# KTH-RPL/neural_graph_mapping

Hardware: AMD Instinct MI355X
Metric: ray-samples/sec (train step: fwd+loss+bwd+Adam, 4096 rays x 128 samples per GPU) (higher is better)
Workload: dtype f32 via 3xbf16 split, fp32 accumulate (hidden-layer matrix products, forward and backward); everything else f32; 1 GPU; M1: 8 fields x 512 rays x (64 coarse + 64 depth-guided) samples per GPU, Fourier(64,raw)+2x64 MLP, nrgbd compositing, NRGBD intrinsics; fields_per_gpu=8, rays_per_field=512, samples_per_ray=128, ranks_seen=1, spin_up_steps=200, jitter=in-kernel Philox, launch=hipGraph replay

## Files before the change

### include/ngm_hip.h

```cpp
#ifndef NGM_HIP_H
#define NGM_HIP_H

#include <stdint.h>

#ifdef __cplusplus
extern "C" {
#endif

#define NGM_ABI_VERSION 11
#define NGM_MAX_LAYERS 4
#define NGM_NUM_LOSS_SUMS 16

enum ngm_status {
  NGM_OK = 0,
  NGM_E_INVALID = -1,
  NGM_E_UNSUPPORTED = -2,
  NGM_E_WORKSPACE = -3,
  NGM_E_HIP = -4
};

enum ngm_encoding { NGM_ENC_NONE = 0, NGM_ENC_FOURIER = 1, NGM_ENC_NERF = 2, NGM_ENC_PERMUTO = 3, NGM_ENC_TRIPLANE = 4 };
enum ngm_triplane_mode { NGM_TRI_SUM = 0, NGM_TRI_PRODUCT = 1, NGM_TRI_CONCAT = 2 };
enum ngm_skip_mode { NGM_SKIP_NO = 0, NGM_SKIP_ADD = 1, NGM_SKIP_CONCAT = 2 };
enum ngm_matmul_mode { NGM_MATMUL_F32 = 0, NGM_MATMUL_BF16X3 = 1, NGM_MATMUL_AUTO = 2 };
// ... 429 lines not shown
                   int32_t width, int32_t height, float fx, float fy, float cx, float cy, float near, float far, float* depth,
                   void* stream);
int ngm_mesh_visibility(const float* verts, int64_t num_verts, const float* c2w, int64_t num_poses, int32_t width, int32_t height,
                        float fx, float fy, float cx, float cy, const float* depth, float eps, int64_t num_frustum_poses,
                        int32_t* in_frustum, int32_t* observed, void* stream);

int64_t ngm_mesh_subdivide_workspace(int64_t num_faces);
int ngm_mesh_subdivide_count(const float* verts, int64_t num_verts, const int64_t* faces, int64_t num_faces, double max_edge,
                             int32_t max_iter, void* workspace, int64_t workspace_bytes, int64_t* totals_dev, void* stream);
int ngm_mesh_subdivide_emit(const float* verts, int64_t num_verts, const int64_t* faces, int64_t num_faces, const float* attrs,
                            int32_t num_channels, const void* workspace, int64_t new_vertices, int64_t out_faces, float* out_verts,
                            int64_t* out_faces_idx, float* out_attrs, int64_t* out_parent, void* stream);

int64_t ngm_mesh_vertex_normals_workspace(int64_t num_verts);
int ngm_mesh_vertex_normals(const float* verts, int64_t num_verts, const int64_t* faces, int64_t num_faces, float* normals,
                            void* workspace, int64_t workspace_bytes, void* stream);
int64_t ngm_icp_point_to_plane_workspace(int64_t num_target, int64_t num_source);
int ngm_icp_point_to_plane(const float* source, int64_t num_source, const float* target, const float* target_normals,
                           int64_t num_target, double threshold, int32_t max_iteration, double relative_fitness,
                           double relative_rmse, const double* init, double* state, void* workspace, int64_t workspace_bytes,
                           void* stream);

int64_t ngm_image_metrics_workspace(int32_t batch, int32_t height, int32_t width, int32_t crop);
int ngm_image_metrics(const float* pred, const float* target, int32_t batch, int32_t height, int32_t width, int32_t crop,
                      double* out, void* workspace, int64_t workspace_bytes, void* stream);

#define NGM_COVER_MAX_NEW 65536
typedef struct ngm_cover_depth_args {
  const float* depth;
  const float* c2w;
  const float* shift;
  const float* field_positions;
  const int64_t* field_ids;
  float* new_positions;
  int32_t* counts;
  int32_t pixel_stride;
  int32_t rows, num_active;
  int32_t height, width;
  int32_t max_new;
  float fx, fy, cx, cy;
  float radius, cell;
} ngm_cover_depth_args;
int64_t ngm_cover_depth_workspace(int32_t height, int32_t width, int32_t num_active, int32_t max_new);
int ngm_cover_depth(const ngm_cover_depth_args* a, void* workspace, int64_t workspace_bytes, void* stream);
int ngm_cover_depth_counters(int32_t height, int32_t width, int32_t num_active, int32_t max_new, void* workspace, int32_t* out5,
                             void* stream);

enum ngm_kernel_id {
  NGM_K_RENDER_FWD = 0,
  NGM_K_STASH_BWD = 1,
  NGM_K_FIELD_BWD = 2,
  NGM_K_GRAD_REDUCE = 3,
  NGM_K_ADAM = 4,
  NGM_K_POINTS_FWD = 5,
  NGM_K_COMPOSITE_FWD = 6,
  NGM_K_COMPOSITE_BWD = 7,
  NGM_K_HASH_GRAD = 8,
  NGM_K_HASH_REDUCE = 9,
  NGM_K_LOSS_REDUCE = 10,
  NGM_K_KNN_ASSIGN = 11,
  NGM_K_KNN_EVAL = 12,
  NGM_K_SAMPLER = 13,
  NGM_K_COUNT = 14
};
int ngm_profile_enable(int32_t on);
int ngm_profile_reset(void);
int ngm_profile_read(int32_t kernel_id, double* total_ms, int64_t* launches);

int ngm_debug_phase_cycles(unsigned long long* out528);
int ngm_debug_fwd_phase_cycles(unsigned long long* out528);

int ngm_debug_last_bwd_variant(void);
int ngm_debug_last_matmul(int which);
int ngm_debug_last_fwd_one_tile(void);
int ngm_debug_last_comp_fused(void);
int ngm_debug_disable_fused_comp(int on);
int ngm_debug_stash_mode(int mode);
int ngm_debug_last_stash_mode(void);
int ngm_debug_plan_bwd(const ngm_field_cfg* fcfg, const ngm_render_cfg* rcfg, int32_t F, int64_t n, int32_t guided,
                       int32_t stash_offered, int32_t seeds_written, int32_t* out5);
int ngm_debug_plan_fwd(const ngm_field_cfg* fcfg, const ngm_render_cfg* rcfg, int32_t surface, int32_t F, int64_t n, int32_t guided,
                       int32_t* out12);

#define NGM_MAX_PEERS 8
typedef struct ngm_peer_exchange {
  int32_t world, rank;
  void* mailbox[NGM_MAX_PEERS];
  unsigned long long* seq;
  int32_t* status;
} ngm_peer_exchange;
int64_t ngm_peer_mailbox_bytes(void);
int ngm_peer_alloc(int64_t bytes, void** ptr);
int ngm_peer_free(void* ptr);
int ngm_ipc_export(void* ptr, unsigned char handle[64]);
int ngm_ipc_open(const unsigned char handle[64], void** ptr);
int ngm_ipc_close(void* ptr);
int ngm_loss_exchange(const ngm_peer_exchange* px, float* loss_sums , void* stream);
double ngm_peer_set_timeout(double seconds);

#ifdef __cplusplus
}
#endif
#endif
```

### neural_graph_mapping_amd/_capi.py

```python
import ctypes as C
import os

HERE = os.path.dirname(os.path.abspath(__file__))
LIB_PATH = os.environ.get("NGM_LIB_PATH") or os.path.join(HERE, "lib", "libngm_hip.so")

NGM_MAX_LAYERS = 4
NGM_NUM_LOSS_SUMS = 16
ENC = {"none": 0, "fourier": 1, "nerf": 2, "permuto": 3, "triplane": 4}
TRI = {"sum": 0, "product": 1, "concat": 2}
SCALE = {"no": 0, "unit_ball": 1, "unit_cube": 2}
GEO = {"nrgbd": 0, "occupancy": 1, "density": 2, "neus": 3}
PHOTO = {"l1": 0, "l2": 1, "gaussian_nll": 2}
DEPTH = {"huber": 0, "gaussian_nll": 1, "laplacian_nll": 2}
LS = dict(PHOTO_SUM=0, PHOTO_CNT=1, DEPTH_SUM=2, DEPTH_CNT=3, FS_SUM=4, FS_CNT=5, TSDF_SUM=6,
          TSDF_CNT=7, TERM_SUM=8, TERM_CNT=9, PHOTO_L1_SUM=10)

f32p = C.c_void_p
LArr = C.c_void_p * (NGM_MAX_LAYERS + 1)
SArr = C.c_int64 * (NGM_MAX_LAYERS + 1)


class FieldCfg(C.Structure):
    _fields_ = [("encoding", C.c_int32), ("dim_enc", C.c_int32), ("raw_coords", C.c_int32),
                ("num_octaves", C.c_int32), ("start_octave", C.c_int32), ("num_layers", C.c_int32),
# ... 265 lines not shown
    L.ngm_render_eval_knn_workspace.argtypes = [P(RenderCfg), i32, i32, i32]
    L.ngm_render_eval_knn_workspace.restype = i64
    L.ngm_target_visibility.argtypes = [P(Keyframes), i32, vp, i32, vp, f32, vp, vp, vp]
    L.ngm_target_rays.argtypes = [P(Keyframes), i32, i32, vp, f32, vp, vp, vp, P(TargetOut), vp]
    L.ngm_target_visibility.restype = C.c_int
    L.ngm_target_rays.restype = C.c_int
    L.ngm_target_sv_intersect.argtypes = [i32, i64, vp, vp, f32, vp, vp]
    L.ngm_target_sv_intersect.restype = C.c_int
    L.ngm_target_sv_rays.argtypes = [i32, i32, vp, f32, vp, vp, vp, i32, i32, f32, f32, f32, f32, P(TargetOut), vp]
    L.ngm_target_sv_rays.restype = C.c_int
    L.ngm_target_sample_mv_workspace.argtypes = [i32, i32, i32, i32]
    L.ngm_target_sample_mv_workspace.restype = i64
    L.ngm_target_sample_mv.argtypes = [P(Keyframes), P(TargetSample), P(TargetOut), vp, i64, vp]
    L.ngm_target_sample_mv.restype = C.c_int
    L.ngm_target_sample_mv_live_workspace.argtypes = [i32, i32, i32, i32]
    L.ngm_target_sample_mv_live_workspace.restype = i64
    L.ngm_target_sample_mv_live.argtypes = [P(Keyframes), P(TargetSample), P(TargetLive), P(TargetOut), vp, i64, vp]
    L.ngm_target_sample_mv_live.restype = C.c_int
    L.ngm_target_observed_fields_workspace.argtypes = [i32, i32]
    L.ngm_target_observed_fields_workspace.restype = i64
    L.ngm_target_observed_fields.argtypes = [P(ObservedFields), vp, i64, vp]
    L.ngm_target_observed_fields.restype = C.c_int
    L.ngm_field_counts_add.argtypes = [vp, vp, i32, vp, i32, vp]
    L.ngm_field_counts_add.restype = C.c_int
    L.ngm_fields_append.argtypes = [P(FieldsAppendArgs), vp]
    L.ngm_fields_append.restype = C.c_int
    L.ngm_fields_repose.argtypes = [P(FieldsReposeArgs), vp]
    L.ngm_fields_repose.restype = C.c_int
    L.ngm_target_sample_mv_grow_workspace.argtypes = [i32, i32, i32, i32]
    L.ngm_target_sample_mv_grow_workspace.restype = i64
    L.ngm_target_sample_mv_grow.argtypes = [P(Keyframes), P(TargetSample), P(TargetLive), vp, P(TargetOut), vp, i64, vp]
    L.ngm_target_sample_mv_grow.restype = C.c_int
    L.ngm_target_observed_fields_grow_workspace.argtypes = [i32, i32]
    L.ngm_target_observed_fields_grow_workspace.restype = i64
    L.ngm_target_observed_fields_grow.argtypes = [P(ObservedFields), vp, vp, i64, vp]
    L.ngm_target_observed_fields_grow.restype = C.c_int
    L.ngm_marching_cubes_workspace.argtypes = [i32, i32, i32]
    L.ngm_marching_cubes_workspace.restype = i64
    L.ngm_marching_cubes_count.argtypes = [vp, i32, i32, i32, f32, vp, vp, i64, vp]
    L.ngm_marching_cubes_emit.argtypes = [vp, i32, i32, i32, f32, vp, i64, vp, i64, vp, i64, vp]
    L.ngm_marching_cubes_tables.argtypes = [vp, vp]
    for name in ("ngm_marching_cubes_count", "ngm_marching_cubes_emit", "ngm_marching_cubes_tables"):
        getattr(L, name).restype = C.c_int
    L.ngm_surface_sample_workspace.argtypes = [i64]
    L.ngm_surface_sample_workspace.restype = i64
    L.ngm_surface_sample.argtypes = [vp, i64, vp, i64, i64, C.c_uint64, vp, vp, vp, i64, vp]
    L.ngm_surface_sample.restype = C.c_int
    L.ngm_nearest_point_workspace.argtypes = [i64, i64]
    L.ngm_nearest_point_workspace.restype = i64
    L.ngm_nearest_point.argtypes = [vp, i64, vp, i64, vp, vp, vp, i64, vp]
    L.ngm_nearest_point.restype = C.c_int
    L.ngm_mesh_depth.argtypes = [vp, i64, vp, i64, vp, i64, i32, i32, f32, f32, f32, f32, f32, f32, vp, vp]
    L.ngm_mesh_depth.restype = C.c_int
    L.ngm_mesh_visibility.argtypes = [vp, i64, vp, i64, i32, i32, f32, f32, f32, f32, vp, f32, i64, vp, vp, vp]
    L.ngm_mesh_visibility.restype = C.c_int
    L.ngm_mesh_subdivide_workspace.argtypes = [i64]
    L.ngm_mesh_subdivide_workspace.restype = i64
    L.ngm_mesh_subdivide_count.argtypes = [vp, i64, vp, i64, C.c_double, i32, vp, i64, vp, vp]
    L.ngm_mesh_subdivide_count.restype = C.c_int
    L.ngm_mesh_subdivide_emit.argtypes = [vp, i64, vp, i64, vp, i32, vp, i64, i64, vp, vp, vp, vp, vp]
    L.ngm_mesh_subdivide_emit.restype = C.c_int
    L.ngm_mesh_vertex_normals_workspace.argtypes = [i64]
    L.ngm_mesh_vertex_normals_workspace.restype = i64
    L.ngm_mesh_vertex_normals.argtypes = [vp, i64, vp, i64, vp, vp, i64, vp]
    L.ngm_mesh_vertex_normals.restype = C.c_int
    L.ngm_icp_point_to_plane_workspace.argtypes = [i64, i64]
    L.ngm_icp_point_to_plane_workspace.restype = i64
    L.ngm_icp_point_to_plane.argtypes = [vp, i64, vp, vp, i64, C.c_double, i32, C.c_double, C.c_double, vp, vp, vp, i64, vp]
    L.ngm_icp_point_to_plane.restype = C.c_int
    L.ngm_image_metrics_workspace.argtypes = [i32, i32, i32, i32]
    L.ngm_image_metrics_workspace.restype = i64
    L.ngm_image_metrics.argtypes = [vp, vp, i32, i32, i32, i32, vp, vp, i64, vp]
    L.ngm_image_metrics.restype = C.c_int
    L.ngm_cover_depth_workspace.argtypes = [i32, i32, i32, i32]
    L.ngm_cover_depth_workspace.restype = i64
    L.ngm_cover_depth.argtypes = [P(CoverDepthArgs), vp, i64, vp]
    L.ngm_cover_depth.restype = C.c_int
    L.ngm_cover_depth_counters.argtypes = [i32, i32, i32, i32, vp, P(i32), vp]
    L.ngm_cover_depth_counters.restype = C.c_int
    L.ngm_debug_plan_bwd.argtypes = [P(FieldCfg), P(RenderCfg), i32, i64, i32, i32, i32, P(i32)]
    L.ngm_debug_plan_bwd.restype = C.c_int
    L.ngm_debug_plan_fwd.argtypes = [P(FieldCfg), P(RenderCfg), i32, i32, i64, i32, P(i32)]
    L.ngm_debug_plan_fwd.restype = C.c_int
    L.ngm_profile_enable.argtypes = [i32]
    L.ngm_profile_read.argtypes = [i32, P(C.c_double), P(i64)]
    for name in ("ngm_profile_enable", "ngm_profile_reset", "ngm_profile_read"):
        getattr(L, name).restype = C.c_int
    for name in ("ngm_sample_rays", "ngm_field_eval_fwd", "ngm_field_eval_bwd", "ngm_composite_fwd",
                 "ngm_composite_bwd", "ngm_render_fwd", "ngm_render_bwd", "ngm_render_bwd_seeded",
                 "ngm_render_read_samples", "ngm_adam_sparse", "ngm_field_eval_knn", "ngm_device_info"):
        getattr(L, name).restype = C.c_int
    _lib = L
    return L


EXPORTED = ["ngm_abi_version", "ngm_last_error", "ngm_device_info", "ngm_permuto_fill_scales", "ngm_sample_rays", "ngm_sample_rays_world", "ngm_sample_rays_weighted",
            "ngm_composite_fwd_packed",
            "ngm_field_eval_fwd", "ngm_encode_fwd", "ngm_encode_bwd", "ngm_encode_bwd_workspace", "ngm_field_eval_bwd", "ngm_field_eval_bwd_workspace",
            "ngm_field_eval_stash_bytes", "ngm_field_eval_fwd_train", "ngm_field_eval_bwd_stash",
            "ngm_composite_fwd", "ngm_composite_bwd", "ngm_render_workspace", "ngm_render_fwd",
            "ngm_render_bwd", "ngm_render_bwd_adam", "ngm_render_bwd_seeded", "ngm_render_bwd_seeded_vars", "ngm_render_read_samples", "ngm_adam_sparse",
            "ngm_field_eval_knn", "ngm_field_eval_knn_workspace", "ngm_grid_eval_knn", "ngm_grid_eval_knn_workspace", "ngm_render_eval_knn", "ngm_render_eval_knn_workspace", "ngm_adam_sparse_multi", "ngm_step_advance", "ngm_profile_enable", "ngm_profile_reset", "ngm_profile_read",
            "ngm_debug_phase_cycles", "ngm_debug_fwd_phase_cycles", "ngm_debug_last_bwd_variant", "ngm_debug_last_matmul", "ngm_debug_last_fwd_one_tile", "ngm_debug_last_comp_fused", "ngm_debug_disable_fused_comp", "ngm_debug_stash_mode", "ngm_debug_last_stash_mode", "ngm_debug_plan_bwd", "ngm_debug_plan_fwd", "ngm_target_visibility", "ngm_target_rays", "ngm_target_sv_intersect", "ngm_target_sv_rays",
            "ngm_target_sample_mv_workspace", "ngm_target_sample_mv",
            "ngm_target_sample_mv_live_workspace", "ngm_target_sample_mv_live", "ngm_target_observed_fields_workspace",
            "ngm_target_observed_fields", "ngm_field_counts_add",
            "ngm_fields_append", "ngm_fields_repose", "ngm_target_sample_mv_grow_workspace", "ngm_target_sample_mv_grow",
            "ngm_target_observed_fields_grow_workspace", "ngm_target_observed_fields_grow",
            "ngm_render_fwd_counted", "ngm_render_bwd_counted", "ngm_render_bwd_adam_counted",
            "ngm_peer_mailbox_bytes", "ngm_peer_alloc", "ngm_peer_free", "ngm_ipc_export", "ngm_ipc_open", "ngm_ipc_close", "ngm_loss_exchange", "ngm_peer_set_timeout",
            "ngm_marching_cubes_workspace", "ngm_marching_cubes_count", "ngm_marching_cubes_emit", "ngm_marching_cubes_tables",
            "ngm_surface_sample_workspace", "ngm_surface_sample", "ngm_nearest_point_workspace", "ngm_nearest_point",
            "ngm_mesh_depth", "ngm_mesh_visibility",
            "ngm_mesh_subdivide_workspace", "ngm_mesh_subdivide_count", "ngm_mesh_subdivide_emit",
            "ngm_mesh_vertex_normals_workspace", "ngm_mesh_vertex_normals", "ngm_icp_point_to_plane_workspace", "ngm_icp_point_to_plane",
            "ngm_image_metrics_workspace", "ngm_image_metrics",
            "ngm_cover_depth_workspace", "ngm_cover_depth", "ngm_cover_depth_counters"]

NO_GRAD_PARAMS = frozenset({"_encoding.random_shift_per_level"})

KERNEL_IDS = dict(render_fwd=0, stash_bwd=1, field_bwd=2, grad_reduce=3, adam=4, points_fwd=5, composite_fwd=6,
                  composite_bwd=7, hash_grad=8, hash_reduce=9, loss_reduce=10, knn_assign=11, knn_eval=12, sampler=13)


NGM_OK, NGM_E_INVALID, NGM_E_UNSUPPORTED, NGM_E_WORKSPACE, NGM_E_HIP = 0, -1, -2, -3, -4


class NgmError(RuntimeError):

    def __init__(self, msg, code=None):
        super().__init__(msg)
        self.code = code


def check(rc, what=""):
    if rc != 0:
        msg = lib().ngm_last_error().decode(errors="replace")
        raise NgmError(f"{what} failed with status {rc}: {msg}", code=int(rc))


SKIP = {"no": 0, "add": 1, "concat": 2}
STASH = {"full": 0, "half": 1}
HASH_ATOMICS = {"exact": 0, "float": 1}
MATMUL = {"f32": 0, "bf16x3": 1, "auto": 2}


def field_cfg(encoding="fourier", dim_enc=64, raw_coords=True, num_octaves=8, start_octave=0,
              num_layers=2, dim_hidden=None, dim_out=4, scale_mode="unit_cube", field_radius=1.0,
              nr_levels=16, nr_feat_per_level=2, log2_hashmap_size=12, coarsest_scale=1.0, finest_scale=1e-4,
              skip_mode="no", matmul_mode="f32", resolution=32, num_components=64, tri_mode="sum"):
    if skip_mode not in SKIP:
        raise NotImplementedError(f"skip_mode={skip_mode!r}: 'no', 'add' and 'concat' have kernels; the reference's own "
                                  "constructor raises for 'rezero' (models.py:131-132)")
    if encoding == "nerf":
        dim_enc = 6 * num_octaves
    if encoding == "none":
        dim_enc = 3
    if encoding == "permuto":
        dim_enc = nr_levels * nr_feat_per_level
    if encoding == "triplane":
        dim_enc = num_components * (3 if tri_mode == "concat" else 1)
    if dim_hidden is None:
        dim_hidden = dim_enc
    fc = FieldCfg(ENC[encoding], dim_enc, int(bool(raw_coords)), num_octaves, start_octave,
                  num_layers, dim_hidden, dim_out, SCALE[scale_mode], float(field_radius), nr_levels,
                  nr_feat_per_level, log2_hashmap_size, float(coarsest_scale), float(finest_scale))
    fc.skip_mode = SKIP[skip_mode]
    fc.matmul_mode = MATMUL[matmul_mode]
    fc.tri_resolution, fc.tri_mode = int(resolution), TRI[tri_mode]
    if encoding == "permuto":
        import math
        import numpy as np
        sig = np.geomspace(coarsest_scale, finest_scale, num=nr_levels)
        for lvl in range(min(nr_levels, 16)):
            for i in range(3):
                fc.level_scale[3 * lvl + i] = np.float32((1.0 / math.sqrt((i + 1) * (i + 2))) / sig[lvl])
    return fc


def param_names(fc: FieldCfg):
    names = []
    if fc.encoding == ENC["fourier"]:
        names.append("_encoding._linear.weight")
    if fc.encoding == ENC["permuto"]:
        names += ["_encoding.lattice_values", "_encoding.random_shift_per_level"]
    if fc.encoding == ENC["triplane"]:
# ... 77 lines not shown
```

### neural_graph_mapping_amd/csrc/ngm_api.hip

```cpp
#include <hip/hip_runtime.h>
#include <stdio.h>
#include <stdlib.h>
#include <string.h>

#include "../../include/ngm_hip.h"
#include "ngm_launch.h"
#include "ngm_workspace.h"

int ngm_launch_sampler_weighted(const ngm_render_cfg* rc, const ngm_rays* rays, int S, int B, const float* boundaries,
                                const float* weights, float* points_cam, float* distances, float* dirs, hipStream_t st);
int ngm_launch_sampler(const ngm_render_cfg* rc, const ngm_rays* rays, int S, float* points_cam, float* distances,
                       float* dirs, float* points_world, hipStream_t st);
int ngm_launch_loss_values(const ngm_render_cfg* rc, const float* sums, float* out, hipStream_t st);
int ngm_launch_loss_reduce(const float* partials, int nblocks, float* sums, uint64_t* counter, hipStream_t st);
int ngm_launch_neus_sd_grad(const float* d_isd_rays, int F, int R, const float* neus_sd, int64_t sd_stride,
                            const int64_t* field_index, float* d_sd, hipStream_t st);
int ngm_launch_read_stash(const float4* sa, const float2* sb, int64_t n, float* geoms, float* dists, hipStream_t st);
int ngm_launch_adam(float* param, float* m, float* v, int64_t stride, const float* grad, int64_t gstride, int F, int64_t numel,
                    const AdamHyper& h, hipStream_t st);
int ngm_launch_adam_multi(const ngm_adam_tensor* tensors, int n, int F, const AdamHyper& h, int64_t* advance_step,
                          uint64_t* advance_offset, hipStream_t st, const int32_t* num_active = nullptr);
int ngm_launch_step_advance(int64_t* step_dev, uint64_t* off_dev, hipStream_t st);
int64_t ngm_mc_workspace_bytes(int nx, int ny, int nz);
int ngm_launch_mc_count(const float* vol, int nx, int ny, int nz, float iso, int64_t* counts, void* workspace,
// ... 658 lines not shown

int ngm_encode_fwd(const ngm_field_cfg* fcfg, const ngm_params* params, int32_t F, int64_t P, const float* points,
                   const float* field_pos, const float* field_quat, float* out, void* stream) {
  int rc = check_field_cfg(fcfg, false);
  if (rc) return rc;
  rc = check_params(fcfg, params);
  if (rc) return rc;
  if (!points || !out || F < 1 || P < 0) return fail(NGM_E_INVALID, "ngm_encode_fwd: bad argument");
  if ((field_pos == nullptr) != (field_quat == nullptr)) return fail(NGM_E_INVALID, "pos/quat must both be given");
  if (P == 0) return NGM_OK;
  rc = ngm_launch_encode_points(*fcfg, *params, F, P, points, field_pos, field_quat, out, (hipStream_t)stream);
  if (rc) return fail(rc, "ngm_encode_fwd: encoding not available as a standalone stage (triplane)");
  return check_launch("ngm_encode_fwd");
}

static int64_t tri_numel(const ngm_field_cfg* fc) {
  const int64_t C = fc->tri_mode == NGM_TRI_CONCAT ? fc->dim_enc / 3 : fc->dim_enc;
  return 3 * C * fc->tri_resolution * fc->tri_resolution;
}
static void hash_scratch_layout(const ngm_field_cfg* fc, int F, int64_t P, FieldBwdArgs& a, WsArena& ws) {
  if (fc->encoding == NGM_ENC_TRIPLANE) { a.tri_numel = tri_numel(fc); a.tri_acc = ws.take<long long>((int64_t)F * a.tri_numel); return; }
  if (fc->encoding != NGM_ENC_PERMUTO) return;
  a.hash_dE = ws.take<float2>((int64_t)fc->nr_levels * F * P);
  a.hash_xyz = ws.take<float4>((int64_t)F * P);
  a.hash_part = ws.take<float>((int64_t)F * fc->nr_levels * 8 * 2 * ((int64_t)1 << fc->log2_hashmap_size));
}

static void encode_bwd_layout(const ngm_field_cfg* fc, int F, int64_t P, float** fourier_part, FieldBwdArgs& a, WsArena& ws) {
  if (fc->encoding == NGM_ENC_FOURIER) *fourier_part = ws.take<float>(ngm_encode_bwd_fourier_scratch(F, P) / 4);
  if (fc->encoding == NGM_ENC_PERMUTO) hash_scratch_layout(fc, F, P, a, ws);
}
int64_t ngm_encode_bwd_workspace(const ngm_field_cfg* fcfg, int32_t F, int64_t P) {
  if (!fcfg || F < 1 || P < 0) return NGM_E_INVALID;
  float* fourier_part;
  return ws_bytes(encode_bwd_layout, fcfg, F, P, &fourier_part, FieldBwdArgs());
}

int ngm_encode_bwd(const ngm_field_cfg* fcfg, const ngm_params* params, int32_t F, int64_t P, const float* points,
                   const float* field_pos, const float* field_quat, const float* d_enc, const ngm_grads* grads, void* workspace,
                   int64_t workspace_bytes, void* stream) {
  int rc = check_field_cfg(fcfg, false);
  if (rc) return rc;
  rc = check_params(fcfg, params);
  if (rc) return rc;
  if (!points || !d_enc || !grads || F < 1 || P < 0) return fail(NGM_E_INVALID, "ngm_encode_bwd: bad argument");
  if ((field_pos == nullptr) != (field_quat == nullptr)) return fail(NGM_E_INVALID, "pos/quat must both be given");
  if (fcfg->encoding == NGM_ENC_TRIPLANE)
    return fail(NGM_E_UNSUPPORTED, "ngm_encode_bwd: the triplane encoding has no standalone backward stage (ngm_field_eval_bwd)");
  if (fcfg->encoding != NGM_ENC_PERMUTO && fcfg->encoding != NGM_ENC_FOURIER) return NGM_OK;
  FieldBwdArgs a;
  memset(&a, 0, sizeof(a));
  float* fourier_part = nullptr;
  WsArena ws(workspace);
  encode_bwd_layout(fcfg, F, P, &fourier_part, a, ws);
  if (!workspace || !ws.covers(workspace_bytes)) return fail(NGM_E_WORKSPACE, "ngm_encode_bwd: workspace too small");
  hipStream_t st = (hipStream_t)stream;
  if (fcfg->encoding == NGM_ENC_FOURIER) {
    if (!grads->enc_w) return fail(NGM_E_INVALID, "ngm_encode_bwd: grads->enc_w is NULL");
    if (P == 0) {
      const int64_t n = (int64_t)(fcfg->dim_enc - (fcfg->raw_coords ? 3 : 0)) * 3;
      for (int f = 0; f < F; ++f) (void)hipMemsetAsync(grads->enc_w + f * grads->enc_w_stride, 0, 4 * (size_t)n, st);
      return check_launch("ngm_encode_bwd");
    }
    rc = ngm_launch_encode_bwd_fourier(*fcfg, *params, F, P, points, field_pos, field_quat, d_enc, grads->enc_w, grads->enc_w_stride,
                                       fourier_part, st);
    if (rc) return fail(rc, "ngm_encode_bwd: launch failed");
    return check_launch("ngm_encode_bwd");
  }
  if (!grads->lattice) return fail(NGM_E_INVALID, "ngm_encode_bwd: grads->lattice is NULL");
  if (!ngm_hash_grad_takes(*fcfg)) return fail(NGM_E_UNSUPPORTED, "ngm_encode_bwd: table size not supported by the table-gradient kernel");
  a.fc = *fcfg; a.pr = *params; a.F = F; a.P = P;
  a.lattice_grad = grads->lattice; a.lattice_grad_stride = grads->lattice_stride;
  if (P == 0) {
    const int64_t n = (int64_t)fcfg->nr_levels * ((int64_t)1 << fcfg->log2_hashmap_size) * 2;
    for (int f = 0; f < F; ++f) (void)hipMemsetAsync(grads->lattice + f * grads->lattice_stride, 0, 4 * (size_t)n, st);
    return check_launch("ngm_encode_bwd");
  }
  rc = ngm_launch_encode_bwd_prep_hash(*fcfg, *params, F, P, points, field_pos, field_quat, d_enc, a.hash_dE, a.hash_xyz, st);
  if (!rc) rc = ngm_launch_hash_grad(a, st);
  if (rc) return fail(rc, "ngm_encode_bwd: table size not supported by the table-gradient kernel");
  return check_launch("ngm_encode_bwd");
}

static int64_t param_pad(const ngm_field_cfg* fc) {
  int64_t e, w[NGM_MAX_LAYERS + 1], b[NGM_MAX_LAYERS + 1];
  return align_up(ngm_param_offsets(fc, &e, w, b), 64);
}

static void field_eval_bwd_layout(const ngm_field_cfg* fc, int64_t P, FieldBwdArgs& a, WsArena& ws) {
  a.partials = ws.take<float>((int64_t)a.F * a.blocks_per_field * a.p_pad + 64);
  hash_scratch_layout(fc, a.F, P, a, ws);
}
int64_t ngm_field_eval_bwd_workspace(const ngm_field_cfg* fcfg, int32_t F, int64_t P) {
  if (check_field_cfg(fcfg)) return NGM_E_INVALID;
  FieldBwdArgs a = FieldBwdArgs();
  int64_t per;
  a.F = F; a.p_pad = param_pad(fcfg);
  plan_bwd(F, P, &per, &a.blocks_per_field);
  return ws_bytes(field_eval_bwd_layout, fcfg, P, a);
}

static BwdPlan plan_points(const ngm_field_cfg* fc, int32_t F, int64_t P, bool stash_offered) { return plan_mlp_bwd(fc, BwdAsk{nullptr, F, P, false, stash_offered}); }
static float* field_eval_stash_layout(const ngm_field_cfg* fc, int32_t F, int64_t P, int64_t* layer_stride, WsArena& ws) {
  *layer_stride = align_up((int64_t)F * P, 32) * 64 + 2048;
  return ws.take<float>(fc->num_layers * *layer_stride + 16);
}
int64_t ngm_field_eval_stash_bytes(const ngm_field_cfg* fcfg, int32_t F, int64_t P) {
  if (check_field_cfg(fcfg) || F < 1 || P < 0) return NGM_E_INVALID;
  if (P == 0 || !plan_points(fcfg, F, P, true).stash_kind) return 0;
  int64_t stride;
  return ws_bytes(field_eval_stash_layout, fcfg, F, P, &stride);
}
static int field_eval_fwd(const ngm_field_cfg* fcfg, const ngm_params* params, int32_t F, int64_t P,
                          const float* points, const float* field_pos, const float* field_quat, float* out, bool stash_offered,
                          void* stash, int64_t stash_bytes, void* stream) {
  int rc = check_field_cfg(fcfg);
  if (rc) return rc;
  rc = check_params(fcfg, params);
  if (rc) return rc;
  if (!points || !out || F < 1 || P < 0) return fail(NGM_E_INVALID, "ngm_field_eval_fwd: bad argument");
  if ((field_pos == nullptr) != (field_quat == nullptr)) return fail(NGM_E_INVALID, "pos/quat must both be given");
  if (P == 0) return NGM_OK;
  FwdAsk ask;
  ask.surface = NGM_FWD_POINTS; ask.F = F; ask.n = P;
  const FwdPlan plan = plan_fwd(fcfg, ask);
  if (plan.status) return fail(plan.status, plan.why);
  PointsFwdArgs a;
  memset(&a, 0, sizeof(a));
  a.fc = *fcfg; a.pr = *params; a.F = F; a.P = P; a.points = points; a.pos = field_pos; a.quat = field_quat; a.out = out;
  if (stash_offered) {
    if (ngm_field_eval_stash_bytes(fcfg, F, P) <= 0) return fail(NGM_E_UNSUPPORTED, "ngm_field_eval_fwd_train: no stash-reading backward for this configuration (ngm_field_eval_stash_bytes == 0): use ngm_field_eval_fwd / ngm_field_eval_bwd");
    WsArena ss(stash);
    a.act = field_eval_stash_layout(fcfg, F, P, &a.act_layer_stride, ss);
    if (!stash || !ss.covers(stash_bytes)) return fail(NGM_E_WORKSPACE, "ngm_field_eval_fwd_train: stash too small (ngm_field_eval_stash_bytes)");
  }
  a.per_block = plan.per_block;
  rc = ngm_launch_points_fwd(a, plan, (hipStream_t)stream);
  if (rc) return fail(rc, no_instance);
  g_last_fwd[NGM_FWD_POINTS] = plan;
  return check_launch("ngm_field_eval_fwd");
}
int ngm_field_eval_fwd(const ngm_field_cfg* fcfg, const ngm_params* params, int32_t F, int64_t P, const float* points,
                       const float* field_pos, const float* field_quat, float* out, void* stream) {
  return field_eval_fwd(fcfg, params, F, P, points, field_pos, field_quat, out, false, nullptr, 0, stream);
}
int ngm_field_eval_fwd_train(const ngm_field_cfg* fcfg, const ngm_params* params, int32_t F, int64_t P, const float* points,
                             const float* field_pos, const float* field_quat, float* out, void* stash, int64_t stash_bytes,
                             void* stream) {
  return field_eval_fwd(fcfg, params, F, P, points, field_pos, field_quat, out, true, stash, stash_bytes, stream);
}

static int field_eval_bwd(const ngm_field_cfg* fcfg, const ngm_params* params, int32_t F, int64_t P,
                          const float* points, const float* field_pos, const float* field_quat, const float* d_out,
                          const ngm_grads* grads, bool stash_offered, const void* stash, int64_t stash_bytes, void* workspace,
                          int64_t workspace_bytes, void* stream) {
  int rc = check_field_cfg(fcfg);
  if (rc) return rc;
  rc = check_params(fcfg, params);
  if (rc) return rc;
  if (!points || !d_out || !grads || F < 1 || P < 1) return fail(NGM_E_INVALID, "ngm_field_eval_bwd: bad argument");
  if ((field_pos == nullptr) != (field_quat == nullptr)) return fail(NGM_E_INVALID, "pos/quat must both be given");
  const BwdPlan plan = plan_points(fcfg, F, P, stash_offered);
  if (plan.status) return fail(plan.status, plan.why);
  FieldBwdArgs a;
  memset(&a, 0, sizeof(a));
  if (stash_offered) {
    if (!plan.stash_kind) return fail(NGM_E_UNSUPPORTED, "ngm_field_eval_bwd_stash: no stash-reading backward for this configuration");
    WsArena ss(stash);
    a.act = field_eval_stash_layout(fcfg, F, P, &a.act_layer_stride, ss);
    if (!stash || !ss.covers(stash_bytes)) return fail(NGM_E_WORKSPACE, "ngm_field_eval_bwd_stash: stash too small");
  }
  a.F = F; a.blocks_per_field = plan.blocks_per_field; a.p_pad = param_pad(fcfg);
  WsArena ws(workspace);
  field_eval_bwd_layout(fcfg, P, a, ws);
  if (!ws.covers(workspace_bytes) || !workspace) return fail(NGM_E_WORKSPACE, "workspace too small");
  hipStream_t st = (hipStream_t)stream;
  a.fc = *fcfg; a.pr = *params; a.F = F; a.P = P; a.points = points; a.pos = field_pos; a.quat = field_quat;
  a.d_out = reinterpret_cast<const float4*>(d_out);
  a.per_block = plan.per_block;
  rc = check_enc_grads(fcfg, grads, a);
  if (rc) return rc;
  if (a.tri_acc) (void)hipMemsetAsync(a.tri_acc, 0, (size_t)F * a.tri_numel * 8, st);
  rc = launch_mlp_bwd(plan, a, st);
  if (rc) return rc;
  if (fcfg->encoding == NGM_ENC_TRIPLANE) { ngm_launch_tri_finish(a, st); rc = check_launch("ngm_tri_finish"); if (rc) return rc; }
  if (fcfg->encoding == NGM_ENC_PERMUTO) {
    rc = ngm_launch_hash_grad(a, st);
    if (rc) return fail(rc, "permutohedral backward: hash table too large for the LDS-staged scatter");
    rc = check_launch("ngm_hash_grad");
    if (rc) return rc;
  }
  GradReduceArgs g;
  memset(&g.adam, 0, sizeof(g.adam));
  g.fc = *fcfg; g.gr = *grads; g.F = F; g.blocks_per_field = a.blocks_per_field; g.partials = a.partials; g.p_pad = a.p_pad;
  ngm_launch_grad_reduce(g, st);
  return check_launch("ngm_grad_reduce");
}
int ngm_field_eval_bwd(const ngm_field_cfg* fcfg, const ngm_params* params, int32_t F, int64_t P, const float* points,
                       const float* field_pos, const float* field_quat, const float* d_out, const ngm_grads* grads,
                       void* workspace, int64_t workspace_bytes, void* stream) {
  return field_eval_bwd(fcfg, params, F, P, points, field_pos, field_quat, d_out, grads, false, nullptr, 0, workspace, workspace_bytes, stream);
}
int ngm_field_eval_bwd_stash(const ngm_field_cfg* fcfg, const ngm_params* params, int32_t F, int64_t P, const float* points,
                             const float* field_pos, const float* field_quat, const float* d_out, const ngm_grads* grads,
                             const void* stash, int64_t stash_bytes, void* workspace, int64_t workspace_bytes, void* stream) {
  return field_eval_bwd(fcfg, params, F, P, points, field_pos, field_quat, d_out, grads, true, stash, stash_bytes, workspace, workspace_bytes, stream);
}

int ngm_composite_fwd(const ngm_render_cfg* cfg, int64_t N, int32_t S, const float* colors, const float* geoms,
                      const float* dists, const float* depths, const float* neus_isds, float* C, float* D, float* Cvar,
                      float* Dvar, float* term, float* weights, void* stream) {
  if (!cfg || !colors || !geoms || !dists || !depths || N < 0) return fail(NGM_E_INVALID, "ngm_composite_fwd: bad argument");
  if (N == 0) return NGM_OK;
  CompositeArgs a;
  memset(&a, 0, sizeof(a));
  a.rc = *cfg; a.N = N; a.S = S; a.colors = colors; a.geoms = geoms; a.dists = dists; a.depths = depths; a.isds = neus_isds;
  a.C = C; a.D = D; a.Cv = Cvar; a.Dv = Dvar; a.term = term; a.weights = weights;
  const int rc = ngm_launch_composite_fwd(a, (hipStream_t)stream);
  if (rc) return fail(rc, "ngm_composite_fwd: unsupported S (max 1024)");
  return check_launch("ngm_composite_fwd");
}

int ngm_composite_fwd_packed(const ngm_render_cfg* cfg, int64_t N, int32_t S, const float* field_out4, const float* dists,
                             const float* points_cam, float* rgbd, float* Cvar, float* Dvar, float* term, void* stream) {
  if (!cfg || !field_out4 || !dists || !points_cam || N < 0) return fail(NGM_E_INVALID, "ngm_composite_fwd_packed: bad argument");
  if (N == 0) return NGM_OK;
  CompositeArgs a;
  memset(&a, 0, sizeof(a));
  a.rc = *cfg; a.N = N; a.S = S; a.out4 = reinterpret_cast<const float4*>(field_out4); a.pcam = points_cam; a.dists = dists;
  a.rgbd = rgbd; a.Cv = Cvar; a.Dv = Dvar; a.term = term;
  const int rc = ngm_launch_composite_fwd(a, (hipStream_t)stream);
  if (rc) return fail(rc, "ngm_composite_fwd_packed: unsupported S (max 1024)");
  return check_launch("ngm_composite_fwd_packed");
}

int ngm_composite_bwd(const ngm_render_cfg* cfg, int64_t N, int32_t S, const float* colors, const float* geoms,
                      const float* dists, const float* depths, const float* neus_isds, const float* dC, const float* dD,
                      const float* dterm, float* d_colors, float* d_geoms, float* d_neus_isds, void* stream) {
  if (!cfg || !colors || !geoms || !dists || !depths || N < 0) return fail(NGM_E_INVALID, "ngm_composite_bwd: bad argument");
  if (N == 0) return NGM_OK;
  CompositeArgs a;
  memset(&a, 0, sizeof(a));
  a.rc = *cfg; a.N = N; a.S = S; a.colors = colors; a.geoms = geoms; a.dists = dists; a.depths = depths; a.isds = neus_isds;
  a.dC = dC; a.dD = dD; a.dterm = dterm; a.d_colors = d_colors; a.d_geoms = d_geoms; a.d_isds = d_neus_isds;
  const int rc = ngm_launch_composite_bwd(a, (hipStream_t)stream);
  if (rc) return fail(rc, "ngm_composite_bwd: S > 1024");
  return check_launch("ngm_composite_bwd");
}

struct RenderPlan {
  int S;
  FwdPlan fwd;
  BwdPlan bwd;
  int64_t p_pad;
  int64_t off_rayseed;
// ... 121 lines not shown
    a.raytab = reinterpret_cast<float*>(ws + p.off_raytab);
    if (has_tg) a.rayseed = reinterpret_cast<float*>(ws + p.off_rayseed);
    a.stashA = reinterpret_cast<float4*>(ws + p.off_stashA);
    a.stashB = reinterpret_cast<float2*>(ws + p.off_stashB);
    a.loss_partials = reinterpret_cast<float*>(ws + p.off_losspart);
    if (p.act_layer_stride) { a.act = reinterpret_cast<float*>(ws + p.off_act); a.act_layer_stride = p.act_layer_stride; }
    a.act_layers = p.bwd.half;
    static const bool timing = getenv("NGM_PHASE_TIMING") != nullptr;
    if (timing) {
      if (!g_debug_cycles_fwd) { (void)hipMalloc(&g_debug_cycles_fwd, NGM_FWD_DEBUG_WORDS * 8); (void)hipMemset(g_debug_cycles_fwd, 0, NGM_FWD_DEBUG_WORDS * 8); }
      a.debug_cycles = g_debug_cycles_fwd;
    }
  }
  e = ngm_launch_render_fwd(a, p.fwd, (hipStream_t)stream);
  if (e) return fail(e, no_instance);
  g_last_fwd[NGM_FWD_RENDER] = p.fwd;
  if (save) {
    note_forward_stash(workspace, p.bwd.half);
    note_forward_seeds(workspace, a.rayseed ? targets->rgbds : nullptr);
  }
  e = check_launch("ngm_render_fwd");
  if (e) return e;
  if (has_tg && loss_sums) {
    ngm_launch_loss_reduce(a.loss_partials, p.fwd.blocks, loss_sums,
                           (rays->philox_offset_autoinc && rays->philox_offset_dev) ? const_cast<uint64_t*>(rays->philox_offset_dev) : nullptr,
                           (hipStream_t)stream);
    e = check_launch("ngm_loss_reduce");
  }
  return e;
}
int ngm_render_fwd(const ngm_field_cfg* fcfg, const ngm_render_cfg* rcfg, const ngm_params* params, const ngm_rays* rays,
                   const ngm_targets* targets, const ngm_prediction* pred, float* loss_sums, void* workspace,
                   int64_t workspace_bytes, void* stream) {
  return render_fwd_impl(fcfg, rcfg, params, rays, targets, pred, loss_sums, workspace, workspace_bytes, stream, nullptr);
}
int ngm_render_fwd_counted(const ngm_field_cfg* fcfg, const ngm_render_cfg* rcfg, const ngm_params* params, const ngm_rays* rays,
                           const ngm_targets* targets, const ngm_prediction* pred, float* loss_sums, void* workspace,
                           int64_t workspace_bytes, void* stream, const int32_t* num_active) {
  const int e = check_counted("ngm_render_fwd_counted", fcfg, rcfg, num_active);
  if (e) return e;
  return render_fwd_impl(fcfg, rcfg, params, rays, targets, pred, loss_sums, workspace, workspace_bytes, stream, num_active);
}

static int render_bwd_common(const ngm_field_cfg* fcfg, const ngm_render_cfg* rcfg, const ngm_params* params,
                             const ngm_rays* rays, StashBwdArgs& sb, const ngm_grads* grads, void* workspace,
                             int64_t workspace_bytes, hipStream_t st, const GradAdam* adam = nullptr,
                             const GradAdam* lattice_adam = nullptr, bool* lattice_adam_applied = nullptr,
                             const int32_t* num_active = nullptr) {
  BwdAsk ask;
  ask.seeded = sb.seed_mode != 0; ask.rec_layers = forward_stash_layers(workspace); ask.seeds_written = forward_wrote_seeds_for(workspace, sb.tg.rgbds);
  FieldBwdArgs a;
  memset(&a, 0, sizeof(a));
  const RenderPlan p = plan_render(fcfg, rcfg, rays->F, rays->R, rays->gt != nullptr, true, ask, false, workspace, &a);
  if (p.bwd.status) return fail(p.bwd.status, p.bwd.why);
  if (!workspace || workspace_bytes < p.total) return fail(NGM_E_WORKSPACE, "render_bwd: workspace too small");
  const bool nll_loss = rcfg->photometric_mode == NGM_PHOTO_GAUSSIAN_NLL || rcfg->depth_mode != NGM_DEPTH_HUBER;
  if (nll_loss && sb.seed_mode == 0 && (!sb.pred.color_vars || !sb.pred.depth_vars))
    return fail(NGM_E_INVALID, "render_bwd: the *_nll loss modes need pred.color_vars and pred.depth_vars");
  char* ws = p.base;
  a.fc = *fcfg; a.pr = *params; a.F = rays->F; a.P = (int64_t)rays->R * p.S; a.S = p.S;
  a.num_active = num_active;
  int e = check_enc_grads(fcfg, grads, a);
  if (e) return e;
  sb.rc = *rcfg; sb.F = rays->F; sb.R = rays->R; sb.S = p.S;
  sb.num_active = num_active;
  if (!rays->gt) sb.rc.w_freespace = sb.rc.w_tsdf = 0.f;
  sb.stashA = reinterpret_cast<float4*>(ws + p.off_stashA);
  sb.stashB = reinterpret_cast<const float2*>(ws + p.off_stashB);
  sb.raytab = reinterpret_cast<const float*>(ws + p.off_raytab);
  const bool neus = rcfg->geometry_mode == NGM_GEO_NEUS;
  if (neus) {
    sb.neus_sd = params->neus_sd; sb.neus_sd_stride = params->neus_sd_stride; sb.field_index = params->field_index;
    sb.d_out = reinterpret_cast<float4*>(ws + p.off_dout);
    sb.d_isd_rays = reinterpret_cast<float*>(ws + p.off_disd);
  }
  if (sb.seed_mode == 0 && !sb.loss_sums) {
    sb.loss_partials = reinterpret_cast<const float*>(ws + p.off_losspart);
    sb.n_partials = p.fwd.blocks;
    sb.counter = (rays->philox_offset_autoinc && rays->philox_offset_dev)
                     ? reinterpret_cast<unsigned long long*>(const_cast<uint64_t*>(rays->philox_offset_dev)) : nullptr;
  }
  a.per_block = p.bwd.per_block; a.blocks_per_field = p.bwd.blocks_per_field;
  a.raytab = sb.raytab; a.stashB = sb.stashB; a.d_out = neus ? sb.d_out : sb.stashA;
  a.partials = reinterpret_cast<float*>(ws + p.off_gradpart); a.p_pad = p.p_pad;
  if (p.bwd.stash_kind) { a.act = reinterpret_cast<const float*>(ws + p.off_act); a.act_layer_stride = p.act_layer_stride; a.act_half = p.bwd.half; }
  if (p.bwd.fused_comp) {
    a.fused_comp = 1; a.rc = sb.rc;
    a.rayseed = reinterpret_cast<const float*>(ws + p.off_rayseed);
    a.loss_sums = sb.loss_sums; a.loss_partials = sb.loss_partials; a.n_partials = sb.n_partials;
    a.sums_out = sb.sums_out; a.loss_out = sb.loss_out; a.counter = sb.counter;
  } else {
    sb.xyz_out = a.hash_xyz;
    a.hash_xyz_ready = a.hash_xyz != nullptr;
    e = ngm_launch_stash_bwd(sb, st);
    if (e) return fail(e, "render_bwd: unsupported geometry mode");
    e = check_launch("ngm_stash_bwd");
    if (e) return e;
  }
  if (neus && grads->neus_sd)
    ngm_launch_neus_sd_grad(sb.d_isd_rays, rays->F, rays->R, params->neus_sd, params->neus_sd_stride, params->field_index,
                            grads->neus_sd, st);
  if (a.tri_acc) (void)hipMemsetAsync(a.tri_acc, 0, (size_t)a.F * a.tri_numel * 8, st);
  e = launch_mlp_bwd(p.bwd, a, st);
  if (e) return e;
  if (fcfg->encoding == NGM_ENC_TRIPLANE) { ngm_launch_tri_finish(a, st); e = check_launch("ngm_tri_finish"); if (e) return e; }
  GradReduceArgs g;
  memset(&g.adam, 0, sizeof(g.adam));
  if (adam) g.adam = *adam;
  g.num_active = num_active;
  g.fc = *fcfg; g.gr = *grads; g.F = rays->F; g.blocks_per_field = a.blocks_per_field; g.partials = a.partials; g.p_pad = a.p_pad;
  bool mlp_reduced = false;
  if (fcfg->encoding == NGM_ENC_PERMUTO) {
    if (lattice_adam) a.lattice_adam = *lattice_adam;
    e = ngm_launch_hash_grad(a, st, lattice_adam_applied, &g, &mlp_reduced);
    if (e == NGM_E_INVALID) return fail(e, "render_bwd_adam: adam tensors do not match the parameter segments");
    if (e) return fail(e, "permutohedral backward: hash table too large for the LDS-staged scatter");
    e = check_launch("ngm_hash_grad");
    if (e) return e;
  }
  if (mlp_reduced) return NGM_OK;
  if (ngm_launch_grad_reduce(g, st)) return fail(NGM_E_INVALID, "render_bwd_adam: adam tensors do not match the parameter segments");
  return check_launch("ngm_grad_reduce");
}

static int render_bwd_impl(const ngm_field_cfg* fcfg, const ngm_render_cfg* rcfg, const ngm_params* params, const ngm_rays* rays,
                           const ngm_targets* targets, const ngm_prediction* pred, const float* loss_sums, const ngm_grads* grads,
                           float* loss_out, void* workspace, int64_t workspace_bytes, void* stream, const int32_t* num_active) {
  int e = check_render(fcfg, rcfg, params, rays);
  if (e) return e;
  if (!targets || !targets->rgbds || !targets->depth_mask || !pred || !pred->rgbds || !pred->term_probs || !grads)
    return fail(NGM_E_INVALID, "render_bwd: NULL argument");
  StashBwdArgs sb;
  memset(&sb, 0, sizeof(sb));
  sb.seed_mode = 0; sb.tg = *targets; sb.pred = *pred; sb.loss_sums = loss_sums;
  sb.loss_out = loss_out;
  return render_bwd_common(fcfg, rcfg, params, rays, sb, grads, workspace, workspace_bytes, (hipStream_t)stream, nullptr, nullptr,
                           nullptr, num_active);
}
int ngm_render_bwd(const ngm_field_cfg* fcfg, const ngm_render_cfg* rcfg, const ngm_params* params, const ngm_rays* rays,
                   const ngm_targets* targets, const ngm_prediction* pred, const float* loss_sums, const ngm_grads* grads,
                   float* loss_out, void* workspace, int64_t workspace_bytes, void* stream) {
  return render_bwd_impl(fcfg, rcfg, params, rays, targets, pred, loss_sums, grads, loss_out, workspace, workspace_bytes, stream,
                         nullptr);
}
int ngm_render_bwd_counted(const ngm_field_cfg* fcfg, const ngm_render_cfg* rcfg, const ngm_params* params, const ngm_rays* rays,
                           const ngm_targets* targets, const ngm_prediction* pred, const float* loss_sums, const ngm_grads* grads,
                           float* loss_out, void* workspace, int64_t workspace_bytes, void* stream, const int32_t* num_active) {
  const int e = check_counted("ngm_render_bwd_counted", fcfg, rcfg, num_active);
  if (e) return e;
  return render_bwd_impl(fcfg, rcfg, params, rays, targets, pred, loss_sums, grads, loss_out, workspace, workspace_bytes, stream,
                         num_active);
}

static int render_bwd_adam_impl(const ngm_field_cfg* fcfg, const ngm_render_cfg* rcfg, const ngm_params* params, const ngm_rays* rays,
                                const ngm_targets* targets, const ngm_prediction* pred, const float* loss_sums, const ngm_grads* grads,
                                const ngm_adam_tensor* mlp_tensors, int32_t num_mlp_tensors, const ngm_adam_tensor* lattice_tensor,
                                const int64_t* field_index, int64_t step, int64_t* step_dev, float lr, float beta1, float beta2,
                                float eps, float weight_decay, float* loss_out, void* workspace, int64_t workspace_bytes,
                                void* stream, const int32_t* num_active) {
  int e = check_render(fcfg, rcfg, params, rays);
  if (e) return e;
  if (!targets || !targets->rgbds || !targets->depth_mask || !pred || !pred->rgbds || !pred->term_probs || !grads ||
      !mlp_tensors || num_mlp_tensors < 1 || (step < 1 && !step_dev))
    return fail(NGM_E_INVALID, "render_bwd_adam: bad argument");
  if ((fcfg->encoding == NGM_ENC_PERMUTO) != (lattice_tensor != nullptr))
    return fail(NGM_E_INVALID, "render_bwd_adam: lattice_tensor goes with the permutohedral encoding");
  StashBwdArgs sb;
// ... 434 lines not shown
      hipStreamSynchronize((hipStream_t)stream) != hipSuccess)
    return check_launch("ngm_cover_depth_counters") == NGM_OK ? fail(NGM_E_HIP, "ngm_cover_depth_counters: copy failed") : NGM_E_HIP;
  return NGM_OK;
}

static int hip_fail(hipError_t e, const char* what) {
  snprintf(g_err, sizeof(g_err), "%s: %s", what, hipGetErrorString(e));
  (void)hipGetLastError();
  return NGM_E_HIP;
}
int64_t ngm_peer_mailbox_bytes(void) { return 2 * NGM_MAX_PEERS * 16 * 8; }
int ngm_peer_alloc(int64_t bytes, void** ptr) {
  if (!ptr || bytes <= 0) return fail(NGM_E_INVALID, "ngm_peer_alloc: bad argument");
  const int e = ngm_peer_alloc_impl(bytes, ptr);
  return e ? hip_fail((hipError_t)e, "ngm_peer_alloc") : NGM_OK;
}
int ngm_peer_free(void* ptr) {
  const hipError_t e = hipFree(ptr);
  return e == hipSuccess ? NGM_OK : hip_fail(e, "ngm_peer_free");
}
int ngm_ipc_export(void* ptr, unsigned char handle[64]) {
  static_assert(sizeof(hipIpcMemHandle_t) == 64, "hipIpcMemHandle_t is 64 bytes");
  if (!ptr || !handle) return fail(NGM_E_INVALID, "ngm_ipc_export: NULL");
  hipIpcMemHandle_t h;
  const hipError_t e = hipIpcGetMemHandle(&h, ptr);
  if (e != hipSuccess) return hip_fail(e, "hipIpcGetMemHandle");
  memcpy(handle, &h, 64);
  return NGM_OK;
}
int ngm_ipc_open(const unsigned char handle[64], void** ptr) {
  if (!ptr || !handle) return fail(NGM_E_INVALID, "ngm_ipc_open: NULL");
  hipIpcMemHandle_t h;
  memcpy(&h, handle, 64);
  const hipError_t e = hipIpcOpenMemHandle(ptr, h, hipIpcMemLazyEnablePeerAccess);
  return e == hipSuccess ? NGM_OK : hip_fail(e, "hipIpcOpenMemHandle");
}
int ngm_ipc_close(void* ptr) {
  const hipError_t e = hipIpcCloseMemHandle(ptr);
  return e == hipSuccess ? NGM_OK : hip_fail(e, "hipIpcCloseMemHandle");
}
int ngm_debug_last_stash_mode(void) { return g_last_bwd.stash_kind ? g_last_bwd.half : -1; }
int ngm_debug_stash_mode(int mode) {
  const int prev = g_stash_override;
  if (mode >= 0 && mode <= 1) g_stash_override = mode;
  else if (mode == -2) g_stash_override = -1;
  return prev;
}

int ngm_debug_plan_bwd(const ngm_field_cfg* fcfg, const ngm_render_cfg* rcfg, int32_t F, int64_t n, int32_t guided,
                       int32_t stash_offered, int32_t seeds_written, int32_t* out5) {
  const int e = check_field_cfg(fcfg);
  if (e) return e;
  if (!out5 || F < 1 || n < 1 || (rcfg && n > INT32_MAX)) return fail(NGM_E_INVALID, "ngm_debug_plan_bwd: bad argument");
  BwdPlan bp;
  int fwd_matmul = -1;
  if (rcfg) {
    BwdAsk ask;
    ask.seeds_written = seeds_written != 0;
    const RenderPlan p = plan_render(fcfg, rcfg, F, (int)n, guided != 0, true, ask);
    bp = p.bwd;
    fwd_matmul = p.fwd.matmul;
  } else {
    bp = plan_points(fcfg, F, n, stash_offered != 0);
  }
  out5[0] = bp.variant; out5[1] = bp.fused_comp; out5[2] = bp.stash_kind; out5[3] = bp.stash_layers; out5[4] = fwd_matmul;
  return bp.status ? fail(bp.status, bp.why) : NGM_OK;
}

int ngm_debug_plan_fwd(const ngm_field_cfg* fcfg, const ngm_render_cfg* rcfg, int32_t surface, int32_t F, int64_t n, int32_t guided,
                       int32_t* out12) {
  const int e = check_field_cfg(fcfg);
  if (e) return e;
  if (!out12 || surface < NGM_FWD_RENDER || surface > NGM_FWD_KNN || (surface == NGM_FWD_RENDER) != (rcfg != nullptr) || F < 1 || n < 1 ||
      (rcfg && n > INT32_MAX))
    return fail(NGM_E_INVALID, "ngm_debug_plan_fwd: bad argument");
  FwdAsk ask;
  ask.surface = surface; ask.F = F; ask.n = n;
  const FwdPlan p = rcfg ? plan_render(fcfg, rcfg, F, (int)n, guided != 0, false).fwd : plan_fwd(fcfg, ask);
  const int32_t out[12] = {p.MI, p.MH, p.L, p.matmul, p.one_tile, p.waves, (int32_t)p.lds_bytes, p.neus, p.threads, p.rays_per_block, p.maxs, p.blocks};
  memcpy(out12, out, sizeof(out));
  return p.status ? fail(p.status, p.why) : NGM_OK;
}

double ngm_peer_set_timeout(double seconds) { return ngm_peer_set_timeout_impl(seconds); }

int ngm_loss_exchange(const ngm_peer_exchange* px, float* loss_sums, void* stream) {
  if (!px || !loss_sums || !px->seq || !px->status) return fail(NGM_E_INVALID, "ngm_loss_exchange: NULL");
  if (px->world < 1 || px->world > NGM_MAX_PEERS || px->rank < 0 || px->rank >= px->world)
    return fail(NGM_E_INVALID, "ngm_loss_exchange: 1 <= world <= 8, 0 <= rank < world");
  for (int p = 0; p < px->world; ++p)
    if (!px->mailbox[p]) return fail(NGM_E_INVALID, "ngm_loss_exchange: mailbox of a rank not mapped");
  ngm_launch_loss_exchange(*px, loss_sums, (hipStream_t)stream);
  return check_launch("ngm_loss_exchange");
}

}
```

### neural_graph_mapping_amd/csrc/ngm_bwd16.h

```cpp
#pragma once
#include "ngm_field.h"
#include "ngm_launch.h"

typedef float f32x4 __attribute__((ext_vector_type(4)));

#define WAVE_SYNC()                                        \
  do {                                                     \
    __builtin_amdgcn_fence(__ATOMIC_RELEASE, "wavefront"); \
    __builtin_amdgcn_wave_barrier();                       \
    __builtin_amdgcn_fence(__ATOMIC_ACQUIRE, "wavefront"); \
  } while (0)

#ifdef NGM_PHASE_TIMING
#define TICK_DECL                                                        \
  unsigned long long tacc[12] = {0, 0, 0, 0, 0, 0, 0, 0, 0, 0, 0, 0};    \
  unsigned long long tlast = __builtin_readcyclecounter();               \
  const unsigned long long tstart = tlast
#define TICK(k)                                                          \
  do {                                                                   \
    if (a.debug_cycles) {                                                \
      const unsigned long long now_ = __builtin_readcyclecounter();      \
      tacc[k] += now_ - tlast; tlast = __builtin_readcyclecounter();     \
    }                                                                    \
  } while (0)
// ... 405 lines not shown
    for (int r = 0; r < 4; ++r)
#pragma unroll
      for (int mi = 0; mi < TIN; ++mi) dX[mi] = mfma16(abuf[mo & 1][mi][r], dY[mo][r], dX[mi]);
    __builtin_amdgcn_sched_barrier(0);
  }
}

template <int TOUT, int TIN>
__device__ __forceinline__ void wgrad16(const float* __restrict__ dbuf, int dstr, const float* __restrict__ xbuf, int xstr,
                                        int lane, f32x4 (&acc)[TOUT][TIN]) {
  const int i = lane & 15, q = lane >> 4;
  const float* dl = dbuf + q * dstr + i;
  const float* xl = xbuf + q * xstr + i;
  float av[2][TOUT], bv[2][TIN];
#pragma unroll
  for (int mo = 0; mo < TOUT; ++mo) av[0][mo] = dl[16 * mo];
#pragma unroll
  for (int mi = 0; mi < TIN; ++mi) bv[0][mi] = xl[16 * mi];
#pragma unroll
  for (int t = 0; t < 4; ++t) {
    if (t + 1 < 4) {
#pragma unroll
      for (int mo = 0; mo < TOUT; ++mo) av[(t + 1) & 1][mo] = dl[4 * (t + 1) * dstr + 16 * mo];
#pragma unroll
      for (int mi = 0; mi < TIN; ++mi) bv[(t + 1) & 1][mi] = xl[4 * (t + 1) * xstr + 16 * mi];
    }
    __builtin_amdgcn_sched_barrier(0);
#pragma unroll
    for (int mo = 0; mo < TOUT; ++mo)
#pragma unroll
      for (int mi = 0; mi < TIN; ++mi) acc[mo][mi] = mfma16(av[t & 1][mo], bv[t & 1][mi], acc[mo][mi]);
    __builtin_amdgcn_sched_barrier(0);
  }
}

template <int T>
__device__ __forceinline__ float colsum16(const float* buf, int stride, int lane) {
  constexpr int NF = 16 * T, PARTS = (64 % NF == 0) ? 64 / NF : 1, PER = 16 / PARTS;
  if (lane >= NF * PARTS) return 0.f;
  const int fl = lane % NF, sp = lane / NF;
  float v[PER];
#pragma unroll
  for (int k = 0; k < PER; ++k) v[k] = buf[(sp * PER + k) * stride + fl];
#pragma unroll
  for (int w = PER / 2; w >= 1; w >>= 1)
#pragma unroll
    for (int k = 0; k < w; ++k) v[k] += v[k + w];
  return v[0];
}
template <int T, int NC>
__device__ __forceinline__ void outer16(const float* colbuf, int stride, const float* row4, int lane, float (&acc)[NC]) {
  constexpr int NF = 16 * T, PARTS = (64 % NF == 0) ? 64 / NF : 1, PER = 16 / PARTS;
  if (lane >= NF * PARTS) return;
  const int fl = lane % NF, sp = lane / NF;
  constexpr int BATCH = (PER < 8) ? PER : 8;
#pragma unroll
  for (int k0 = 0; k0 < PER; k0 += BATCH) {
    float h[BATCH]; float4 d[BATCH];
#pragma unroll
    for (int k = 0; k < BATCH; ++k) { const int s = sp * PER + k0 + k; h[k] = colbuf[s * stride + fl]; d[k] = *reinterpret_cast<const float4*>(row4 + 4 * s); }
#pragma unroll
    for (int k = 0; k < BATCH; ++k) {
      acc[0] = fmaf(d[k].x, h[k], acc[0]); acc[1] = fmaf(d[k].y, h[k], acc[1]); acc[2] = fmaf(d[k].z, h[k], acc[2]);
      if (NC > 3) acc[3] = fmaf(d[k].w, h[k], acc[3]);
    }
  }
}
template <int T>
__device__ __forceinline__ float fold_parts(float v) {
  constexpr int NF = 16 * T;
  if (NF <= 32) v += __shfl_down(v, 32, 64);
  if (NF <= 16) v += __shfl_down(v, 16, 64);
  return v;
}

template <int TI, int TH, int L, bool ENC_GRAD, int EPI_CH = 4>
__device__ __forceinline__ void bwd16_epilogue(const FieldBwdArgs& a, float* stage, f32x4 (&acc0)[TH][TI],
                                               f32x4 (&accH)[(L > 1) ? (L - 1) : 1][TH][TH], float (&dbh)[L],
                                               float (&dwo)[4], float (&dwf)[3], float (&dbo)[4]) {
  const int lane = threadIdx.x & 63, wave = threadIdx.x >> 6;
  int64_t enc_off, w_off[NGM_MAX_LAYERS + 1], b_off[NGM_MAX_LAYERS + 1];
  const int64_t ptot = ngm_param_offsets(&a.fc, &enc_off, w_off, b_off);
  (void)ptot;
  float* dst = a.partials + (int64_t)blockIdx.x * a.p_pad;
  const int D = a.fc.dim_enc, H = a.fc.dim_hidden;
  constexpr int NT0 = TH * TI, NTH = TH * TH, NT = NT0 + (L - 1) * NTH;
  constexpr int EPI_W = EPI_CH * 4 * 64;
#pragma unroll
  for (int t0 = 0; t0 < NT; t0 += EPI_CH) {
#pragma unroll
    for (int tt = 0; tt < EPI_CH; ++tt) {
      const int t = t0 + tt;
      if (t < NT) {
#pragma unroll
        for (int r = 0; r < 4; ++r) {
          float v;
          if (t < NT0) v = acc0[t / TI][t % TI][r];
          else v = accH[(t - NT0) / NTH][((t - NT0) % NTH) / TH][(t - NT0) % TH][r];
          stage[wave * EPI_W + (tt * 4 + r) * 64 + lane] = v;
        }
      }
    }
    __syncthreads();
    for (int e = threadIdx.x; e < EPI_W; e += B16_THREADS) {
      float s0 = 0.f;
#pragma unroll
      for (int w = 0; w < B16_WAVES; ++w) s0 += stage[w * EPI_W + e];
      const int t = t0 + (e >> 8), r = (e >> 6) & 3, jj = e & 15, qq = (e >> 4) & 3;
      if (t < NT) {
        int l, mo, mi, din;
        if (t < NT0) { l = 0; mo = t / TI; mi = t % TI; din = D; }
        else { const int u = t - NT0; l = 1 + u / NTH; mo = (u % NTH) / TH; mi = u % TH; din = H; }
        const int o = 16 * mo + 4 * qq + r, c = 16 * mi + jj;
        if (o < H && c < din) dst[w_off[l] + (int64_t)o * din + c] = s0;
      }
    }
    __syncthreads();
  }
#pragma unroll
  for (int l = 0; l < L; ++l) dbh[l] = fold_parts<TH>(dbh[l]);
#pragma unroll
  for (int c = 0; c < 4; ++c) dwo[c] = fold_parts<TH>(dwo[c]);
#pragma unroll
  for (int c = 0; c < 3; ++c) dwf[c] = fold_parts<TI>(dwf[c]);
#pragma unroll
  for (int c = 0; c < 4; ++c) dbo[c] = wave_sum(dbo[c]);
  constexpr int NV = L + 4 + 3 + 4;
  static_assert(NV * 64 <= EPI_W, "per-feature vectors must fit one staging round");
  {
    float* sw = stage + wave * EPI_W;
#pragma unroll
    for (int l = 0; l < L; ++l) sw[l * 64 + lane] = dbh[l];
#pragma unroll
    for (int c = 0; c < 4; ++c) sw[(L + c) * 64 + lane] = dwo[c];
#pragma unroll
    for (int c = 0; c < 3; ++c) sw[(L + 4 + c) * 64 + lane] = dwf[c];
#pragma unroll
    for (int c = 0; c < 4; ++c) sw[(L + 7 + c) * 64 + lane] = dbo[c];
  }
  __syncthreads();
  const bool fourier = ENC_GRAD && a.fc.encoding == NGM_ENC_FOURIER;
  const int n_raw = a.fc.raw_coords ? 3 : 0;
  for (int e = threadIdx.x; e < NV * 64; e += B16_THREADS) {
    float s0 = 0.f;
#pragma unroll
    for (int w = 0; w < B16_WAVES; ++w) s0 += stage[w * EPI_W + e];
    const int k = e >> 6, ln = e & 63;
    if (k < L) { if (ln < H) dst[b_off[k] + ln] = s0; }
    else if (k < L + 4) { if (ln < H) dst[w_off[L] + (int64_t)(k - L) * H + ln] = s0; }
    else if (k < L + 7) { if (fourier && ln < D && ln >= n_raw) dst[enc_off + (int64_t)(ln - n_raw) * 3 + (k - L - 4)] = s0; }
    else if (ln == 0) dst[b_off[L] + (k - L - 7)] = s0;
  }
  if (!fourier)
    for (int64_t p = enc_off + threadIdx.x; p < w_off[0]; p += B16_THREADS) dst[p] = 0.f;
}
```

### neural_graph_mapping_amd/csrc/ngm_field_bwd.hip

```cpp
#include <stdlib.h>
#include <string.h>
#include <algorithm>
#include "ngm_field.h"
#include "ngm_launch.h"

#define WAVE_SYNC()                                        \
  do {                                                     \
    __builtin_amdgcn_fence(__ATOMIC_RELEASE, "wavefront"); \
    __builtin_amdgcn_wave_barrier();                       \
    __builtin_amdgcn_fence(__ATOMIC_ACQUIRE, "wavefront"); \
  } while (0)

template <int MI, int MH, int L, bool CAT = false>
struct BwdLds {
  using LY = FieldLds<MI, MH, L, CAT>;
  static constexpr int STR_E = 32 * MI + 4;
  static constexpr int STR_H = 32 * MH + 4;
  static constexpr int STR_D = (STR_E > STR_H) ? STR_E : STR_H;
  static constexpr int X0 = 0;
  static constexpr int x_off(int l) { return l == 0 ? 0 : 32 * STR_E + (l - 1) * 32 * STR_H; }
  static constexpr int DBUF = 32 * STR_E + (L - 1) * 32 * STR_H;
  static constexpr int PBUF = DBUF + 32 * STR_D;
  static constexpr int OBUF = PBUF + 128;
  static constexpr int WAVE_TOTAL = OBUF + 128;
// ... 383 lines not shown
#pragma unroll
            for (int r = 0; r < 16; ++r) dY[mi][r] = (Xl[mi][r] > 0.f) ? dX[mi][r] : 0.f;
        }
      }
    }
  }

  __syncthreads();
  float* red = sm + LY::TOTAL;
  int64_t enc_off, w_off[NGM_MAX_LAYERS + 1], b_off[NGM_MAX_LAYERS + 1];
  const int64_t ptot = ngm_param_offsets(&a.fc, &enc_off, w_off, b_off);
  for (int64_t p = threadIdx.x; p < ptot; p += NGM_BLOCK) red[p] = 0.f;
  __syncthreads();
  const int D = a.fc.dim_enc, H = a.fc.dim_hidden;
  if (MH == 1) {
#pragma unroll
    for (int l = 0; l < L; ++l) dbh[l] += __shfl_down(dbh[l], 32, 64);
#pragma unroll
    for (int c = 0; c < 4; ++c) dwo[c] += __shfl_down(dwo[c], 32, 64);
  }
  if (MI == 1) {
#pragma unroll
    for (int c = 0; c < 3; ++c) dwf[c] += __shfl_down(dwf[c], 32, 64);
    if constexpr (CAT) {
#pragma unroll
      for (int c = 0; c < 4; ++c) dwoE[c] += __shfl_down(dwoE[c], 32, 64);
    }
  }
  const int DC = CAT ? H + D : H;
#pragma unroll
  for (int c = 0; c < 4; ++c) dbo[c] = wave_sum(dbo[c]);
  for (int w = 0; w < NGM_WAVES_PER_BLOCK; ++w) {
    if (wave == w) {
#pragma unroll
      for (int mo = 0; mo < MH; ++mo) {
#pragma unroll
        for (int r = 0; r < 16; ++r) {
          const int o = 32 * mo + frow(r, hi);
          if (o < H) {
#pragma unroll
            for (int mi = 0; mi < MI; ++mi) {
              const int i = 32 * mi + j;
              if (i < D) red[w_off[0] + (int64_t)o * D + i] += acc0[mo][mi][r];
            }
#pragma unroll
            for (int l = 1; l < L; ++l) {
#pragma unroll
              for (int mi = 0; mi < MH; ++mi) {
                const int i = 32 * mi + j;
                if (i < H) red[w_off[l] + (int64_t)o * DC + i] += accH[l - 1][mo][mi][r];
              }
              if constexpr (CAT) {
#pragma unroll
                for (int mi = 0; mi < MI; ++mi) {
                  const int i = 32 * mi + j;
                  if (i < D) red[w_off[l] + (int64_t)o * DC + H + i] += accE[l - 1][mo][mi][r];
                }
              }
            }
          }
        }
      }
      if (lane < 32 * MH && lane < H) {
#pragma unroll
        for (int l = 0; l < L; ++l) red[b_off[l] + lane] += dbh[l];
#pragma unroll
        for (int c = 0; c < 4; ++c) red[w_off[L] + (int64_t)c * DC + lane] += dwo[c];
      }
      if (CAT && lane < 32 * MI && lane < D) {
#pragma unroll
        for (int c = 0; c < 4; ++c) red[w_off[L] + (int64_t)c * DC + H + lane] += dwoE[c];
      }
      if (lane < 4) red[b_off[L] + lane] += (lane == 0 ? dbo[0] : lane == 1 ? dbo[1] : lane == 2 ? dbo[2] : dbo[3]);
      if (ENC_GRAD && a.fc.encoding == NGM_ENC_FOURIER) {
        const int n_raw = a.fc.raw_coords ? 3 : 0;
        if (lane < 32 * MI && lane < D && lane >= n_raw) {
#pragma unroll
          for (int c = 0; c < 3; ++c) red[enc_off + (int64_t)(lane - n_raw) * 3 + c] += dwf[c];
        }
      }
    }
    __syncthreads();
  }
  float* dst = a.partials + (int64_t)blockIdx.x * a.p_pad;
  for (int64_t p = threadIdx.x; p < ptot; p += NGM_BLOCK) dst[p] = red[p];
}

struct GradSeg { int64_t off, size; float* dst; int64_t stride; float* param; float* m; float* v; int64_t pstride; void* lp; int lp_dt; };
struct GradReduceK {
  int F, blocks_per_field, nseg;
  const float* partials;
  int64_t p_pad, ptot;
  GradSeg seg[2 * (NGM_MAX_LAYERS + 1) + 1];
  AdamHyper hyper;
  const int32_t* num_active;
};

template <bool COUNTED>
__global__ void __launch_bounds__(256) k_grad_reduce(GradReduceK a) {
  __shared__ float part[4][64];
  const int f = blockIdx.y, q = threadIdx.x >> 6, l = threadIdx.x & 63;
  if constexpr (COUNTED) {
    if (f >= *a.num_active) return;
  }
  const int64_t p = (int64_t)blockIdx.x * 64 + l;
  int seg = -1;
  int64_t so = 0;
  float pv = 0.f, m0 = 0.f, v0 = 0.f;
  AdamCoef co = {0.f, 1.f};
  const bool adam = q == 0 && p < a.ptot;
  if (adam) {
    for (int k = 0; k < a.nseg; ++k)
      if (p >= a.seg[k].off && p < a.seg[k].off + a.seg[k].size) { seg = k; break; }
    if (seg >= 0 && a.seg[seg].param) {
      const int64_t row = a.hyper.field_index ? a.hyper.field_index[f] : f;
      so = row * a.seg[seg].pstride + (p - a.seg[seg].off);
      pv = a.seg[seg].param[so]; m0 = a.seg[seg].m[so]; v0 = a.seg[seg].v[so];
    }
  }
  const float* src = a.partials + (int64_t)f * a.p_pad + p;
  const int64_t cs = (int64_t)a.F * a.p_pad;
  int c = q;
  float v8[8] = {0.f, 0.f, 0.f, 0.f, 0.f, 0.f, 0.f, 0.f};
  const bool pre = p < a.ptot && c + 28 < a.blocks_per_field;
  if (pre) {
#pragma unroll
    for (int j = 0; j < 8; ++j) v8[j] = src[(c + 4 * j) * cs];
  }
  if (adam && seg >= 0 && a.seg[seg].param) {
    const double step = (double)(a.hyper.step_dev ? *a.hyper.step_dev : a.hyper.step);
    co = adam_coef(a.hyper.lr, a.hyper.beta1, a.hyper.beta2, step);
  }
  float s = 0.f;
  if (pre) {
#pragma unroll
    for (int j = 0; j < 8; ++j) s += v8[j];
    c += 32;
  }
  if (p < a.ptot) {
#pragma unroll 1
    for (; c + 28 < a.blocks_per_field; c += 32) {
      float v[8];
#pragma unroll
      for (int j = 0; j < 8; ++j) v[j] = src[(c + 4 * j) * cs];
#pragma unroll
      for (int j = 0; j < 8; ++j) s += v[j];
    }
#pragma unroll 1
    for (; c + 12 < a.blocks_per_field; c += 16) {
      const float v0_ = src[c * cs], v1 = src[(c + 4) * cs], v2 = src[(c + 8) * cs], v3 = src[(c + 12) * cs];
      s += v0_; s += v1; s += v2; s += v3;
    }
    for (; c < a.blocks_per_field; c += 4) s += src[c * cs];
  }
  part[q][l] = s;
  __syncthreads();
  if (q != 0 || p >= a.ptot || seg < 0) return;
  s = ((part[0][l] + part[1][l]) + part[2][l]) + part[3][l];
  const int64_t i = p - a.seg[seg].off;
  if (a.seg[seg].dst) a.seg[seg].dst[(int64_t)f * a.seg[seg].stride + i] = s;
  if (a.seg[seg].param) {
    const float pn = adam_update(pv, m0, v0, s, co, a.hyper.beta1, a.hyper.beta2, a.hyper.eps, a.hyper.wd);
    a.seg[seg].m[so] = m0; a.seg[seg].v[so] = v0;
    a.seg[seg].param[so] = pn;
    if (a.seg[seg].lp) ngm_stp(a.seg[seg].lp, so, pn, a.seg[seg].lp_dt);
  }
}

template <bool COUNTED>
__device__ __forceinline__ void grad_reduce_one(const GradReduceK& a, int f, int64_t p) {
  if (p >= a.ptot) return;
  if constexpr (COUNTED) {
    if (f >= *a.num_active) return;
  }
  int seg = -1;
  for (int k = 0; k < a.nseg; ++k)
    if (p >= a.seg[k].off && p < a.seg[k].off + a.seg[k].size) { seg = k; break; }
  int64_t so = 0;
  float pv = 0.f, m0 = 0.f, v0 = 0.f;
  const bool adam = seg >= 0 && a.seg[seg].param;
  if (adam) {
    const int64_t row = a.hyper.field_index ? a.hyper.field_index[f] : f;
    so = row * a.seg[seg].pstride + (p - a.seg[seg].off);
    pv = a.seg[seg].param[so]; m0 = a.seg[seg].m[so]; v0 = a.seg[seg].v[so];
  }
  const float* src = a.partials + (int64_t)f * a.p_pad + p;
  const int64_t cs = (int64_t)a.F * a.p_pad;
  float q[4] = {0.f, 0.f, 0.f, 0.f};
  if (a.blocks_per_field <= 8) {
    float v[8];
#pragma unroll
    for (int c = 0; c < 8; ++c) v[c] = (c < a.blocks_per_field) ? src[c * cs] : 0.f;
#pragma unroll
    for (int i = 0; i < 4; ++i) {
      float s = 0.f;
      if (i < a.blocks_per_field) s += v[i];
      if (i + 4 < a.blocks_per_field) s += v[i + 4];
      q[i] = s;
    }
  } else {
    for (int c0 = 0; c0 < a.blocks_per_field; c0 += 16) {
      float v[16];
#pragma unroll
      for (int u = 0; u < 16; ++u) v[u] = (c0 + u < a.blocks_per_field) ? src[(int64_t)(c0 + u) * cs] : 0.f;
#pragma unroll
      for (int u = 0; u < 16; ++u)
        if (c0 + u < a.blocks_per_field) q[u & 3] += v[u];
    }
  }
  AdamCoef co = {0.f, 1.f};
  if (adam) {
    const double step = (double)(a.hyper.step_dev ? *a.hyper.step_dev : a.hyper.step);
    co = adam_coef(a.hyper.lr, a.hyper.beta1, a.hyper.beta2, step);
  }
  const float s = ((q[0] + q[1]) + q[2]) + q[3];
  if (seg < 0) return;
  const int64_t i = p - a.seg[seg].off;
  if (a.seg[seg].dst) a.seg[seg].dst[(int64_t)f * a.seg[seg].stride + i] = s;
  if (adam) {
    const float pn = adam_update(pv, m0, v0, s, co, a.hyper.beta1, a.hyper.beta2, a.hyper.eps, a.hyper.wd);
    a.seg[seg].m[so] = m0; a.seg[seg].v[so] = v0;
    a.seg[seg].param[so] = pn;
    if (a.seg[seg].lp) ngm_stp(a.seg[seg].lp, so, pn, a.seg[seg].lp_dt);
  }
}
template <bool COUNTED>
__global__ void __launch_bounds__(256) k_grad_reduce_flat(GradReduceK a) {
  grad_reduce_one<COUNTED>(a, blockIdx.y, (int64_t)blockIdx.x * 256 + threadIdx.x);
}

static int build_grad_reduce(const GradReduceArgs& g, GradReduceK& k) {
  k.F = g.F; k.blocks_per_field = g.blocks_per_field; k.partials = g.partials; k.p_pad = g.p_pad;
  k.num_active = g.num_active;
  int64_t enc_off, w_off[NGM_MAX_LAYERS + 1], b_off[NGM_MAX_LAYERS + 1];
  k.ptot = ngm_param_offsets(&g.fc, &enc_off, w_off, b_off);
  int n = 0;
  if (g.fc.encoding == NGM_ENC_FOURIER) {
    const int64_t sz = (int64_t)(g.fc.raw_coords ? g.fc.dim_enc - 3 : g.fc.dim_enc) * 3;
    k.seg[n++] = GradSeg{enc_off, sz, g.gr.enc_w, g.gr.enc_w_stride, nullptr, nullptr, nullptr, 0, nullptr, 0};
  }
  for (int l = 0; l <= g.fc.num_layers; ++l) {
    const int din = (l == 0) ? g.fc.dim_enc : g.fc.dim_hidden + (g.fc.skip_mode == NGM_SKIP_CONCAT ? g.fc.dim_enc : 0);
    const int dout = (l == g.fc.num_layers) ? g.fc.dim_out : g.fc.dim_hidden;
    k.seg[n++] = GradSeg{w_off[l], (int64_t)din * dout, g.gr.w[l], g.gr.w_stride[l], nullptr, nullptr, nullptr, 0, nullptr, 0};
    k.seg[n++] = GradSeg{b_off[l], (int64_t)dout, g.gr.b[l], g.gr.b_stride[l], nullptr, nullptr, nullptr, 0, nullptr, 0};
  }
  k.nseg = n;
  k.hyper = AdamHyper{nullptr, nullptr, 1, 0.f, 0.f, 0.f, 0.f, 0.f};
  if (g.adam.tensors) {
    if (g.adam.num != n) return NGM_E_INVALID;
    for (int i = 0; i < n; ++i) {
      const ngm_adam_tensor& t = g.adam.tensors[i];
      if (t.numel != k.seg[i].size || !t.param || !t.exp_avg || !t.exp_avg_sq) return NGM_E_INVALID;
      k.seg[i].param = t.param; k.seg[i].m = t.exp_avg; k.seg[i].v = t.exp_avg_sq; k.seg[i].pstride = t.stride;
      k.seg[i].lp = t.param_lp; k.seg[i].lp_dt = t.lp_dtype;
    }
    k.hyper = g.adam.hyper;
  }
  return 0;
}
int ngm_launch_grad_reduce(const GradReduceArgs& g, hipStream_t st) {
  NgmProfScope prof_(NGM_K_GRAD_REDUCE, st);
  GradReduceK k;
  const int rc = build_grad_reduce(g, k);
  if (rc) return rc;
  if (k.blocks_per_field <= 8) {
    dim3 grid((unsigned)((k.ptot + 255) / 256), (unsigned)g.F);
    if (k.num_active) hipLaunchKernelGGL(k_grad_reduce_flat<true>, grid, dim3(256), 0, st, k);
    else hipLaunchKernelGGL(k_grad_reduce_flat<false>, grid, dim3(256), 0, st, k);
    return 0;
  }
  dim3 grid((unsigned)((k.ptot + 63) / 64), (unsigned)g.F);
  if (k.num_active) hipLaunchKernelGGL(k_grad_reduce<true>, grid, dim3(256), 0, st, k);
  else hipLaunchKernelGGL(k_grad_reduce<false>, grid, dim3(256), 0, st, k);
  return 0;
}

template <int MI, int MH, int L>
static int launch_bwd(const FieldBwdArgs& a, int blocks, hipStream_t st) {
#define NGM_LB(NC, EG, HS, CT)                                                                                          \
  do {                                                                                                                  \
    const size_t lds = BwdLds<MI, MH, L, CT>::TOTAL * sizeof(float);                                                    \
    static_assert(BwdLds<MI, MH, L, CT>::TOTAL * sizeof(float) <= NGM_LDS_MAX, "k_field_bwd: LDS over 160 KiB");          \
    (void)hipFuncSetAttribute((const void*)k_field_bwd<MI, MH, L, NC, EG, HS, CT>, hipFuncAttributeMaxDynamicSharedMemorySize, \
                              (int)lds);                                                                                \
    hipLaunchKernelGGL((k_field_bwd<MI, MH, L, NC, EG, HS, CT>), dim3(blocks), dim3(NGM_BLOCK), lds, st, a);            \
  } while (0)
  const bool cat = a.fc.skip_mode == NGM_SKIP_CONCAT;
  if (a.fc.encoding == NGM_ENC_PERMUTO) {
    if constexpr (MI == 1) { if (cat) NGM_LB(false, false, 1, true); else NGM_LB(false, false, 1, false); }
    else return NGM_E_INVALID;
  } else if (a.fc.encoding == NGM_ENC_TRIPLANE) {
    if (!a.tri_acc) return NGM_E_INVALID;
    if (cat) NGM_LB(false, false, 2, true); else NGM_LB(false, false, 2, false);
  } else if (a.fc.encoding == NGM_ENC_FOURIER) { if (cat) NGM_LB(false, true, 0, true); else NGM_LB(false, true, 0, false); }
  else if (a.fc.encoding == NGM_ENC_NERF) { if (cat) NGM_LB(true, false, 0, true); else NGM_LB(true, false, 0, false); }
  else { if (cat) NGM_LB(false, false, 0, true); else NGM_LB(false, false, 0, false); }
#undef NGM_LB
  return 0;
}

__global__ void k_tri_finish(const long long* acc, int64_t numel, float* grad, int64_t gstride) {
  const int f = blockIdx.y;
  for (int64_t i = (int64_t)blockIdx.x * blockDim.x + threadIdx.x; i < numel; i += (int64_t)gridDim.x * blockDim.x)
    grad[(int64_t)f * gstride + i] = (float)((double)acc[(int64_t)f * numel + i] * (1.0 / 1099511627776.0));
}
int ngm_launch_tri_finish(const FieldBwdArgs& a, hipStream_t st) {
  if (!a.tri_acc || !a.planes_grad) return NGM_E_INVALID;
  const int bx = (int)std::min<int64_t>((a.tri_numel + 255) / 256, 1024);
  hipLaunchKernelGGL(k_tri_finish, dim3(bx, a.F), dim3(256), 0, st, a.tri_acc, a.tri_numel, a.planes_grad, a.planes_grad_stride);
  return 0;
}

#ifdef NGM_FAST_BUILD
#define NGM_BWD_INSTANCES(X) X(2, 2, 2)
#else
#define NGM_BWD_INSTANCES(X) X(2, 2, 2) X(2, 2, 1) X(1, 1, 1) X(1, 1, 2)
#endif
bool ngm_field_bwd_takes(const ngm_field_cfg& fc, const BwdProblem& q) {
  const FieldShape s = field_shape(&fc);
  if (q.half || q.fused_comp || (fc.encoding == NGM_ENC_PERMUTO && s.MI != 1)) return false;
#define NGM_X(mi, mh, l) if (s.MI == mi && s.MH == mh && s.L == l) return true;
  NGM_BWD_INSTANCES(NGM_X)
#undef NGM_X
  return false;
}
int ngm_launch_field_bwd(const FieldBwdArgs& a, int blocks, hipStream_t st) {
  if (!ngm_field_bwd_takes(a.fc, bwd_problem(a))) return NGM_E_INVALID;
  NgmProfScope prof_(NGM_K_FIELD_BWD, st);
  const FieldShape s = field_shape(&a.fc);
#define NGM_X(mi, mh, l) if (s.MI == mi && s.MH == mh && s.L == l) return launch_bwd<mi, mh, l>(a, blocks, st);
  NGM_BWD_INSTANCES(NGM_X)
#undef NGM_X
  return NGM_E_INVALID;
}

__device__ __forceinline__ unsigned long long to_fix(float v) {
  const float s = v * 512.0f;
  const float tr = truncf(s);
  const int hi = (int)tr;
  const int lo = (int)((s - tr) * 2147483648.0f);
  const long long r = (long long)hi * 2147483648ll + (long long)lo;
  return (unsigned long long)r;
}

struct HashGradArgs {
  ngm_field_cfg fc;
  ngm_params pr;
  int F; int64_t P; int chunks; int64_t per_chunk;
  const float2* dE; const float4* xyz;
  float* gtab; int64_t gstride;
  float* part;
  float* ad_param; float* ad_m; float* ad_v; int64_t ad_stride; void* ad_lp; int ad_lp_dt;
  AdamHyper hyper;
  int hash_blocks, mlp_bx;
// ... 183 lines not shown

__global__ void k_hash_reduce(HashGradArgs a) {
  const int T = 1 << a.fc.log2_hashmap_size;
  const int level = blockIdx.y, f = blockIdx.z;
  const int i = blockIdx.x * blockDim.x + threadIdx.x;
  if (i >= T / 2) return;
  if (a.num_active && f >= *a.num_active) return;
  const float4* src = reinterpret_cast<const float4*>(a.part + ((int64_t)f * a.fc.nr_levels + level) * a.chunks * 2 * T);
  float4 s = make_float4(0.f, 0.f, 0.f, 0.f);
  for (int c = 0; c < a.chunks; ++c) {
    const float4 v = src[(int64_t)c * (T / 2) + i];
    s.x += v.x; s.y += v.y; s.z += v.z; s.w += v.w;
  }
  reinterpret_cast<float4*>(a.gtab + (int64_t)f * a.gstride + (int64_t)level * T * 2)[i] = s;
  if (a.ad_param) {
    const double step = (double)(a.hyper.step_dev ? *a.hyper.step_dev : a.hyper.step);
    const AdamCoef co = adam_coef(a.hyper.lr, a.hyper.beta1, a.hyper.beta2, step);
    const int64_t row = a.hyper.field_index ? a.hyper.field_index[f] : f;
    const int64_t o4 = (row * a.ad_stride + (int64_t)level * T * 2) / 4 + i;
    float4 p = reinterpret_cast<float4*>(a.ad_param)[o4], m = reinterpret_cast<float4*>(a.ad_m)[o4],
           v = reinterpret_cast<float4*>(a.ad_v)[o4];
    adam_update4(p, m, v, s, co, a.hyper.beta1, a.hyper.beta2, a.hyper.eps, a.hyper.wd);
    reinterpret_cast<float4*>(a.ad_m)[o4] = m; reinterpret_cast<float4*>(a.ad_v)[o4] = v;
    reinterpret_cast<float4*>(a.ad_param)[o4] = p;
    if (a.ad_lp) {
#pragma unroll
      for (int c = 0; c < 4; ++c) ngm_stp(a.ad_lp, 4 * o4 + c, (&p.x)[c], a.ad_lp_dt);
    }
  }
}

static size_t hash_grad_lds(const ngm_field_cfg& fc) {
  const bool flt = fc.hash_grad_atomics == NGM_HASH_ATOMICS_FLOAT;
  return ((size_t)2 << fc.log2_hashmap_size) * (flt ? sizeof(float) : sizeof(unsigned long long));
}
bool ngm_hash_grad_takes(const ngm_field_cfg& fc) { return hash_grad_lds(fc) <= 150 * 1024; }

int ngm_launch_hash_grad(const FieldBwdArgs& fb, hipStream_t st, bool* adam_applied, const GradReduceArgs* mlp_reduce,
                         bool* mlp_reduced) {
  HashGradArgs a;
  a.hash_blocks = 0; a.mlp_bx = 0;
  memset(&a.mlp, 0, sizeof(a.mlp));
  if (mlp_reduced) *mlp_reduced = false;
  a.fc = fb.fc; a.pr = fb.pr; a.F = fb.F; a.P = fb.P; a.dE = fb.hash_dE; a.xyz = fb.hash_xyz;
  a.gtab = fb.lattice_grad; a.gstride = fb.lattice_grad_stride;
  a.num_active = fb.num_active;
  const int T = 1 << fb.fc.log2_hashmap_size;
  const bool flt = fb.fc.hash_grad_atomics == NGM_HASH_ATOMICS_FLOAT;
  const size_t lds = hash_grad_lds(fb.fc);
  if (!ngm_hash_grad_takes(fb.fc)) return NGM_E_UNSUPPORTED;
  const int units = (int)fb.F * fb.fc.nr_levels;
  constexpr int NT = 512;
  int ncu = 256;
  {
    int dev = 0;
    hipDeviceProp_t prop;
    static int cached = 0;
    if (!cached && hipGetDevice(&dev) == hipSuccess && hipGetDeviceProperties(&prop, dev) == hipSuccess && prop.multiProcessorCount > 0)
      cached = prop.multiProcessorCount;
    if (cached) ncu = cached;
  }
  const int slots = 2 * ncu;
  int chunks = (int)((slots + (int64_t)units - 1) / (int64_t)units);
  const int64_t max_chunks = (fb.P + 4095) / 4096;
  if (chunks > max_chunks) chunks = (int)max_chunks;
  if (chunks < 1) chunks = 1;
  if (chunks > 8) chunks = 8;
  a.chunks = chunks; a.per_chunk = (fb.P + chunks - 1) / chunks;
  a.part = fb.hash_part;
  a.ad_param = nullptr; a.ad_lp = nullptr; a.ad_lp_dt = 0;
  if (fb.lattice_adam.tensors) {
    const ngm_adam_tensor& t = fb.lattice_adam.tensors[0];
    const int64_t per = (int64_t)fb.fc.nr_levels * T * 2;
    if (t.numel == per && (t.stride & 3) == 0 &&
        ((reinterpret_cast<uintptr_t>(t.param) | reinterpret_cast<uintptr_t>(t.exp_avg) | reinterpret_cast<uintptr_t>(t.exp_avg_sq)) & 15) == 0) {
      a.ad_param = t.param; a.ad_m = t.exp_avg; a.ad_v = t.exp_avg_sq; a.ad_stride = t.stride;
      a.ad_lp = t.param_lp; a.ad_lp_dt = t.lp_dtype;
      a.hyper = fb.lattice_adam.hyper;
    }
  }
  a.hash_blocks = chunks * units;
  if (mlp_reduce) {
    if (build_grad_reduce(*mlp_reduce, a.mlp)) return NGM_E_INVALID;
    a.mlp_bx = (int)((a.mlp.ptot + NT - 1) / NT);
    if (mlp_reduced) *mlp_reduced = true;
  }
  const int grid_x = a.hash_blocks + a.mlp_bx * (int)fb.F;
  {
    NgmProfScope prof_(NGM_K_HASH_GRAD, st);
#define NGM_HG(FLT_)                                                                                                          \
    do {                                                                                                                      \
      (void)hipFuncSetAttribute((const void*)k_hash_grad<FLT_, 1, NT>, hipFuncAttributeMaxDynamicSharedMemorySize, (int)lds); \
      hipLaunchKernelGGL((k_hash_grad<FLT_, 1, NT>), dim3(grid_x), dim3(NT), lds, st, a);                                    \
    } while (0)
    if (flt) NGM_HG(true); else NGM_HG(false);
#undef NGM_HG
  }
  if (chunks > 1) {
    NgmProfScope prof_(NGM_K_HASH_REDUCE, st);
    hipLaunchKernelGGL(k_hash_reduce, dim3((T / 2 + 255) / 256, fb.fc.nr_levels, fb.F), dim3(256), 0, st, a);
  }
  if (adam_applied) *adam_applied = a.ad_param != nullptr;
  return 0;
}
```

### neural_graph_mapping_amd/csrc/ngm_field_bwd_b3.hip

```cpp
#include "ngm_bwd_b3.h"

template <bool NEED_COS, bool ENC_GRAD>
__device__ __forceinline__ void recompute_with_encoding(const ngm_u32x4* __restrict__ P, const float* __restrict__ tile,
                                                        const float* __restrict__ pb, const float4 (&encw)[2], int lane,
                                                        f32x16 (&Hc)[2], float (&Eb)[2][2][8], float (&Cb)[2][2][8]) {
  const int hi = lane >> 5;
  const float inv2pi = 0.15915494309189535f;
  const f32x16 zero = {0.f, 0.f, 0.f, 0.f, 0.f, 0.f, 0.f, 0.f, 0.f, 0.f, 0.f, 0.f, 0.f, 0.f, 0.f, 0.f};
  RowRegs R;
  PlaneRegs W[2];
  float4 pq[2][4];
  load_rows(tile, lane, R);
  load_planes(P, 0, lane, W[0]);
  auto ldq = [&](int q) __attribute__((always_inline)) {
#pragma unroll
    for (int j = 0; j < 4; ++j) {
      const int b = q >> 1, e = 4 * (q & 1) + j;
      pq[q & 1][j] = *reinterpret_cast<const float4*>(pb + 4 * (8 * ((8 * b + e) >> 2) + 4 * hi + (e & 3)));
    }
  };
  ldq(0);
  __builtin_amdgcn_sched_barrier(0);
  B3Op A = b3_rows(R.g[0][0], R.g[0][1]);
  __builtin_amdgcn_sched_barrier(0);
// ... 561 lines not shown
#ifdef NGM_ABLB_NOENC
          Eb[b][m][e] = p.x + w.x;
          if (ENC_GRAD) dwf[m][0] += dE[m][8 * b + e];
          continue;
#endif
          const float arg = fmaf(w.z, p.z, fmaf(w.y, p.y, w.x * p.x));
          const float rev = __builtin_amdgcn_fractf(arg * inv2pi);
          const float sn = __builtin_amdgcn_sinf(rev);
          float v = sn;
          if (NEED_COS) v = (w.w == NGM_FK_COS) ? __builtin_amdgcn_cosf(rev) : sn;
          if (m == 0) v = (w.w == NGM_FK_RAW) ? arg : v;
          Eb[b][m][e] = v;
          if (ENC_GRAD) {
            const float g = dE[m][8 * b + e] * __builtin_amdgcn_cosf(rev);
            dwf[m][0] = fmaf(g, p.x, dwf[m][0]); dwf[m][1] = fmaf(g, p.y, dwf[m][1]); dwf[m][2] = fmaf(g, p.z, dwf[m][2]);
          }
        }
      }
      __builtin_amdgcn_sched_barrier(0);
    }
    }
    if constexpr (HS && ENC_GRAD) {
      accl[192] = make_float4(dwf[0][0], dwf[0][1], dwf[0][2], 0.f);
      accl[256] = make_float4(dwf[1][0], dwf[1][1], dwf[1][2], 0.f);
    }
    WAVE_SYNC();
    TICK(3);
    if constexpr (FC) {
      if (it + 2u < ntiles) issue_small(base - 64u, (int)(it & 1u));
    }
    if (more) {
      if constexpr (!FC) {
        if (pts) {
          issue_inputs_pts(fs.dout, pts_base, nxt, end, lane, wl_lds + LY::INB * 4, wl_lds + LY::INB * 4 + 2048);
          issue_inputs_pts(fs.dout, pts_base, nxt + 16, end, lane, wl_lds + LY::INB * 4 + 1024, wl_lds + LY::INB * 4 + 2048 + 256);
        } else {
          issue_inputs(fs, a.S, nxt, end, lane, wl_lds + LY::INB * 4);
          issue_inputs(fs, a.S, nxt + 16, end, lane, wl_lds + LY::INB * 4 + 1024);
        }
      }
      const uint32_t u0 = nxt + fs.gb;
      if (((u0 & 31u) == 0u) && (nxt + 32u <= end)) {
        if constexpr (!HS) issue_tile32_fast(fs.act[L - 1], u0 >> 5, lane, wl_lds + LY::HL * 4);
        if (L == 2) issue_tile32_fast(fs.act[0], u0 >> 5, lane, wl_lds + LY::H1 * 4);
      } else {
        if constexpr (!HS) issue_tile32(fs.act[L - 1], fs.gb, nxt, end, lane, wl_lds + LY::HL * 4);
        if (L == 2) issue_tile32(fs.act[0], fs.gb, nxt, end, lane, wl_lds + LY::H1 * 4);
      }
    }
    __builtin_amdgcn_sched_barrier(0);
    TICK(5);
    {
      B3Op A0[2] = {b3_regs<0>(dY[0]), b3_regs<0>(dY[1])}, B0[2] = {b3_arr(Eb[0][0]), b3_arr(Eb[0][1])};
      __builtin_amdgcn_sched_barrier(0);
      B3Op A1[2] = {b3_regs<1>(dY[0]), b3_regs<1>(dY[1])}, B1[2] = {b3_arr(Eb[1][0]), b3_arr(Eb[1][1])};
      wgrad_b3_block_free(A0, B0, acc[0]);
      NGM_INTERLEAVE(24, 8)
      __builtin_amdgcn_sched_barrier(0);
      wgrad_b3_block(A1, B1, acc[0]);
    }
    __builtin_amdgcn_sched_barrier(0);
    TICK(10);
    DMA_WAIT(0);
    TICK(2);
    WAVE_SYNC();
  }
#undef COL_OFF
  PTK(6);
  if constexpr (HS) {
    const float4 a0 = accl[0], a1 = accl[64], a2 = accl[128], f0 = accl[192], f1 = accl[256];
    dwo[0][0] = a0.x; dwo[0][1] = a0.y; dwo[0][2] = a0.z; dwo[0][3] = a0.w;
    dwo[1][0] = a1.x; dwo[1][1] = a1.y; dwo[1][2] = a1.z; dwo[1][3] = a1.w;
    dbh[L - 1][0] = a2.x; dbh[L - 1][1] = a2.y; dbh[0][0] = a2.z; dbh[0][1] = a2.w;
    dwf[0][0] = f0.x; dwf[0][1] = f0.y; dwf[0][2] = f0.z;
    dwf[1][0] = f1.x; dwf[1][1] = f1.y; dwf[1][2] = f1.z;
  }
  __syncthreads();

  float* stage = sm;
  constexpr int NT = LY::NT;
  constexpr int NV = 2 * L + 8 + 6 + 4;
  static_assert(LY::EPI_ACC + B3B_WAVES * NV * 64 <= LY::TOTAL, "the per-feature vectors are staged behind the accumulator tiles");
  float* stagev = sm + LY::EPI_ACC;
#pragma unroll
  for (int l = 0; l < L; ++l)
#pragma unroll
    for (int mo = 0; mo < 2; ++mo)
#pragma unroll
      for (int mi = 0; mi < 2; ++mi)
#pragma unroll
        for (int q = 0; q < 4; ++q) {
          const f32x16& c = acc[l][mo][mi];
          *reinterpret_cast<float4*>(stage + (((wave * NT + (l * 4 + mo * 2 + mi)) * 4 + q) * 64 + lane) * 4) =
              make_float4(c[4 * q], c[4 * q + 1], c[4 * q + 2], c[4 * q + 3]);
        }
  {
    float* sw = stagev + wave * NV * 64;
    int k = 0;
#pragma unroll
    for (int l = 0; l < L; ++l)
#pragma unroll
      for (int m = 0; m < 2; ++m) sw[(k++) * 64 + lane] = dbh[l][m];
#pragma unroll
    for (int m = 0; m < 2; ++m)
#pragma unroll
      for (int c = 0; c < 4; ++c) sw[(k++) * 64 + lane] = dwo[m][c];
#pragma unroll
    for (int m = 0; m < 2; ++m)
#pragma unroll
      for (int c = 0; c < 3; ++c) sw[(k++) * 64 + lane] = dwf[m][c];
#pragma unroll
    for (int c = 0; c < 4; ++c) sw[(k++) * 64 + lane] = wave_sum(dbo[c]);
  }
  __syncthreads();
  int64_t enc_off, w_off[NGM_MAX_LAYERS + 1], b_off[NGM_MAX_LAYERS + 1];
  (void)ngm_param_offsets(&a.fc, &enc_off, w_off, b_off);
  float* dst = a.partials + (int64_t)blockIdx.x * a.p_pad;
  const int D = a.fc.dim_enc, H = a.fc.dim_hidden;
  {
    static_assert(NT * 256 % B3B_THREADS == 0, "whole passes");
    constexpr int NIT = NT * 256 / B3B_THREADS;
    float4 v4[NIT][B3B_WAVES];
#pragma unroll
    for (int it = 0; it < NIT; ++it)
#pragma unroll
      for (int w = 0; w < B3B_WAVES; ++w)
        v4[it][w] = *reinterpret_cast<const float4*>(stage + (w * NT * 256 + it * B3B_THREADS + threadIdx.x) * 4);
#pragma unroll
    for (int it = 0; it < NIT; ++it) {
      const int e4 = it * B3B_THREADS + threadIdx.x;
      float4 s4 = make_float4(0.f, 0.f, 0.f, 0.f);
#pragma unroll
      for (int w = 0; w < B3B_WAVES; ++w) {
        s4.x += v4[it][w].x; s4.y += v4[it][w].y; s4.z += v4[it][w].z; s4.w += v4[it][w].w;
      }
      const int t = e4 >> 8, q = (e4 >> 6) & 3, ln = e4 & 63;
      const int l = t >> 2, mo = (t >> 1) & 1, mi = t & 1;
      const int o0 = 32 * mo + 8 * q + 4 * (ln >> 5), c = 32 * mi + (ln & 31), din = (l == 0) ? D : H;
      if (c < din) {
        float* d = dst + w_off[l] + (int64_t)o0 * din + c;
        if (o0 < H) d[0] = s4.x;
        if (o0 + 1 < H) d[din] = s4.y;
        if (o0 + 2 < H) d[2 * din] = s4.z;
        if (o0 + 3 < H) d[3 * din] = s4.w;
      }
    }
  }
  const bool fourier = ENC_GRAD && a.fc.encoding == NGM_ENC_FOURIER;
  const int n_raw = a.fc.raw_coords ? 3 : 0;
  {
    constexpr int NIV = (NV * 32 + B3B_THREADS - 1) / B3B_THREADS;
    float sv[NIV];
#pragma unroll
    for (int it = 0; it < NIV; ++it) {
      const int e = it * B3B_THREADS + threadIdx.x;
      const int k = min(e >> 5, NV - 1), ii = e & 31;
      float s0 = 0.f;
#pragma unroll
      for (int w = 0; w < B3B_WAVES; ++w) s0 += stagev[(w * NV + k) * 64 + ii] + stagev[(w * NV + k) * 64 + 32 + ii];
      sv[it] = s0;
    }
#pragma unroll
    for (int it = 0; it < NIV; ++it) {
      const int e = it * B3B_THREADS + threadIdx.x;
      if (e >= NV * 32) break;
      const int k = e >> 5, ii = e & 31;
      const float s0 = sv[it];
      if (k < 2 * L) {
        const int l = k >> 1, ft = 32 * (k & 1) + ii;
        if (ft < H) dst[b_off[l] + ft] = s0;
      } else if (k < 2 * L + 8) {
        const int u = k - 2 * L, ft = 32 * (u >> 2) + ii, c = u & 3;
        if (ft < H) dst[w_off[L] + (int64_t)c * H + ft] = s0;
      } else if (k < 2 * L + 14) {
        const int u = k - 2 * L - 8, ft = 32 * (u / 3) + ii, c = u % 3;
        if (fourier && ft < D && ft >= n_raw) dst[enc_off + (int64_t)(ft - n_raw) * 3 + c] = s0;
      } else if (ii == 0) {
        dst[b_off[L] + (k - 2 * L - 14)] = 0.5f * s0;
      }
    }
  }
  if (!fourier)
    for (int64_t p = enc_off + threadIdx.x; p < w_off[0]; p += B3B_THREADS) dst[p] = 0.f;
  TICK(11);
  TICK_REPORT
#ifdef NGM_PROLOGUE_TIMING
  PTK(7);
  if (a.debug_cycles && blockIdx.x == gridDim.x / 2 && threadIdx.x == 0) {
    for (int k = 0; k < 8; ++k) a.debug_cycles[k] = ptk_[k];
    for (int k = 8; k < 13; ++k) a.debug_cycles[k] = 0;
    a.debug_cycles[12] = ptk_[7];
  }
#endif
#undef PTK
}

template <int L, bool HS>
static int launch_bwd_b3(const FieldBwdArgs& a, int blocks, hipStream_t st) {
#define NGM_LBB3(NC, EG)                                                                                              \
  do {                                                                                                                \
    static_assert(LdsB3b<L, EG, HS>::TOTAL * sizeof(float) <= NGM_LDS_MAX, "k_field_bwd_b3: LDS over 160 KiB");       \
    const size_t lds = (size_t)LdsB3b<L, EG, HS>::TOTAL * sizeof(float);                                              \
    if (a.fused_comp) NGM_LBB3_ONE(NC, EG, true); else NGM_LBB3_ONE(NC, EG, false);                                    \
  } while (0)
#define NGM_LBB3_ONE(NC, EG, FC_)                                                                                     \
  do {                                                                                                                \
    if (a.num_active) {                                                                                               \
      (void)hipFuncSetAttribute((const void*)k_field_bwd_b3<L, NC, EG, FC_, HS, true>, hipFuncAttributeMaxDynamicSharedMemorySize, \
                                (int)lds);                                                                            \
      hipLaunchKernelGGL((k_field_bwd_b3<L, NC, EG, FC_, HS, true>), dim3(blocks), dim3(B3B_THREADS), lds, st, a);    \
    } else {                                                                                                          \
      (void)hipFuncSetAttribute((const void*)k_field_bwd_b3<L, NC, EG, FC_, HS>, hipFuncAttributeMaxDynamicSharedMemorySize, \
                                (int)lds);                                                                            \
      hipLaunchKernelGGL((k_field_bwd_b3<L, NC, EG, FC_, HS>), dim3(blocks), dim3(B3B_THREADS), lds, st, a);          \
    }                                                                                                                 \
  } while (0)
  if (a.fc.encoding == NGM_ENC_FOURIER) NGM_LBB3(false, true);
  else if (a.fc.encoding == NGM_ENC_NERF) NGM_LBB3(true, false);
  else NGM_LBB3(false, false);
#undef NGM_LBB3
#undef NGM_LBB3_ONE
  return 0;
}

bool ngm_field_bwd_b3_takes(const ngm_field_cfg& fc, const BwdProblem& q) {
  const int MI = (fc.dim_enc + 31) / 32, MH = (fc.dim_hidden + 31) / 32, L = fc.num_layers;
  if (q.stash_kind != 1 || (q.points && (q.fused_comp || q.half)) || fc.skip_mode != NGM_SKIP_NO || fc.matmul_mode == NGM_MATMUL_F32 || MI != 2 || MH != 2 || L < 1 || L > 2)
    return false;
  if (fc.encoding != NGM_ENC_FOURIER && fc.encoding != NGM_ENC_NERF && fc.encoding != NGM_ENC_NONE) return false;
  if ((q.P + 64) * 256 >= ((int64_t)1 << 32)) return false;
  if (q.half && L != 2) return false;
  if (q.fused_comp && q.per_block % (B3B_WAVES * 32)) return false;
#ifdef NGM_FAST_BUILD
  if (L != 2) return false;
#endif
  return true;
}
int ngm_launch_field_bwd_b3(const FieldBwdArgs& a, int blocks, hipStream_t st) {
  if (!ngm_field_bwd_b3_takes(a.fc, bwd_problem(a)) || (a.fused_comp && !a.rayseed)) return NGM_E_INVALID;
  NgmProfScope prof_(NGM_K_FIELD_BWD, st);
  if (a.fc.num_layers == 2) return a.act_half ? launch_bwd_b3<2, true>(a, blocks, st) : launch_bwd_b3<2, false>(a, blocks, st);
#ifndef NGM_FAST_BUILD
  if (a.fc.num_layers == 1) return launch_bwd_b3<1, false>(a, blocks, st);
#endif
  return NGM_E_INVALID;
}
```

### neural_graph_mapping_amd/csrc/ngm_hash_bwd.hip

```cpp
#include "ngm_bwd_b3.h"

#define HB_WAVES 8
#define HB_THREADS 512
#define HB_PG 128

struct LdsHB {
  static constexpr int PLANES = 2 * 3 * HB_PG * 4;
  static constexpr int CONSTS = PLANES;
  static constexpr int WAVES = CONSTS + 192;
  static constexpr int ET = 0, DT = 1024, OB = 2048;
  static constexpr int WAVE_TOTAL = 2048 + 768;
  static constexpr int BODY = WAVES + HB_WAVES * WAVE_TOTAL;
  static constexpr int EPI = HB_WAVES * 1024 + HB_WAVES * 9 * 64;
  static constexpr int TOTAL = BODY > EPI ? BODY : EPI;
};

__device__ __forceinline__ void hb_issue_tile(const char* sbase, uint32_t gb, uint32_t n0, uint32_t end, int lane, uint32_t lds_tile) {
#pragma unroll
  for (int k = 0; k < 4; ++k) {
    const uint32_t c = 2 * k + (lane >> 5);
    uint32_t n = n0 + (((uint32_t)lane & 31u) ^ (c & 7u));
    if (n >= end) n = end - 1;
    const uint32_t u = n + gb;
    dma16_so(sbase, (((u >> 5) * 8u + c) * 32u + ((u & 31u) ^ (c & 7u))) * 16u, lds_tile + k * 1024);
// ... 287 lines not shown
    }
#pragma unroll
    for (int r = 0; r < 16; ++r) Dt[COL_OFF(r)] = dY[r];
    WAVE_SYNC();
    float4 dr[2][2];
    ngm_u32x4 wd[2][3];
    float Ec[16];
#pragma unroll
    for (int r = 0; r < 16; ++r) Ec[r] = Et[COL_OFF(r)];
#pragma unroll
    for (int kb = 0; kb < 2; ++kb) {
      const int c0 = 4 * kb + 2 * hi;
      dr[kb][0] = *reinterpret_cast<const float4*>(Dt + tile_chunk(c0, i));
      dr[kb][1] = *reinterpret_cast<const float4*>(Dt + tile_chunk(c0 + 1, i));
#pragma unroll
      for (int p = 0; p < 3; ++p) wd[kb][p] = Pd[p * HB_PG + (kb * 2 + hi) * 32 + i];
    }
    WAVE_SYNC();
    if (more) issue(nxt);
    __builtin_amdgcn_sched_barrier(0);
#pragma unroll
    for (int b = 0; b < 2; ++b) {
      float ya[8], xa[8];
#pragma unroll
      for (int e = 0; e < 8; ++e) { ya[e] = dY[8 * b + e]; xa[e] = Ec[8 * b + e]; }
      const B3Op A = b3_arr(ya), Bx = b3_arr(xa);
      acc = mfma_bf16(A.l, Bx.h, acc);
      acc = mfma_bf16(A.h, Bx.l, acc);
      acc = mfma_bf16(A.m, Bx.m, acc);
      acc = mfma_bf16(A.m, Bx.h, acc);
      acc = mfma_bf16(A.h, Bx.m, acc);
      acc = mfma_bf16(A.h, Bx.h, acc);
    }
    f32x16 dE;
#pragma unroll
    for (int r = 0; r < 16; ++r) dE[r] = 0.f;
#pragma unroll
    for (int kb = 0; kb < 2; ++kb) {
      const B3Op Bd = b3_rows(dr[kb][0], dr[kb][1]);
      const ngm_bf16x8 wh = __builtin_bit_cast(ngm_bf16x8, wd[kb][0]), wm = __builtin_bit_cast(ngm_bf16x8, wd[kb][1]),
                       wlo = __builtin_bit_cast(ngm_bf16x8, wd[kb][2]);
      dE = mfma_bf16(wlo, Bd.h, dE);
      dE = mfma_bf16(wh, Bd.l, dE);
      dE = mfma_bf16(wm, Bd.m, dE);
      dE = mfma_bf16(wm, Bd.h, dE);
      dE = mfma_bf16(wh, Bd.m, dE);
      dE = mfma_bf16(wh, Bd.h, dE);
    }
    if (base + (uint32_t)i < end) {
      int li = i, lh = hi;
      asm volatile("" : "+v"(li), "+v"(lh));
      float2* dst = a.hash_dE + (g0 + base + li) + (int64_t)(2 * lh) * NP;
#pragma unroll
      for (int q = 0; q < 4; ++q)
#pragma unroll
        for (int p = 0; p < 2; ++p) {
          const int lv = 4 * q + p;
          if (lv + 2 * hi < nlev) {
            typedef float v2f __attribute__((ext_vector_type(2)));
            const v2f v = {dE[4 * q + 2 * p], dE[4 * q + 2 * p + 1]};
            ngm_store_wt(reinterpret_cast<ngm_v2f_*>(dst + (int64_t)lv * NP), v);
          }
        }
    }
    DMA_WAIT(0);
    WAVE_SYNC();
  }
#undef COL_OFF
  __syncthreads();

  float* stage = sm;
#pragma unroll
  for (int q = 0; q < 4; ++q)
    *reinterpret_cast<float4*>(stage + ((wave * 4 + q) * 64 + lane) * 4) = make_float4(acc[4 * q], acc[4 * q + 1], acc[4 * q + 2], acc[4 * q + 3]);
  float* vec = stage + HB_WAVES * 1024 + wave * 9 * 64;
  vec[lane] = dbh;
#pragma unroll
  for (int c = 0; c < 4; ++c) vec[(1 + c) * 64 + lane] = dwo[c];
#pragma unroll
  for (int c = 0; c < 4; ++c) vec[(5 + c) * 64 + lane] = wave_sum(dbo[c]);
  __syncthreads();
  int64_t enc_off, w_off[NGM_MAX_LAYERS + 1], b_off[NGM_MAX_LAYERS + 1];
  (void)ngm_param_offsets(&a.fc, &enc_off, w_off, b_off);
  float* dstp = a.partials + (int64_t)blockIdx.x * a.p_pad;
  if (threadIdx.x < 256) {
    const int e4 = threadIdx.x;
    float4 s4 = make_float4(0.f, 0.f, 0.f, 0.f);
#pragma unroll
    for (int w = 0; w < HB_WAVES; ++w) {
      const float4 v = *reinterpret_cast<const float4*>(stage + (w * 256 + e4) * 4);
      s4.x += v.x; s4.y += v.y; s4.z += v.z; s4.w += v.w;
    }
    const int q = e4 >> 6, ln = e4 & 63;
    const int o0 = 8 * q + 4 * (ln >> 5), c = ln & 31;
    if (c < D) {
      float* d = dstp + w_off[0] + (int64_t)o0 * D + c;
      if (o0 < H) d[0] = s4.x;
      if (o0 + 1 < H) d[D] = s4.y;
      if (o0 + 2 < H) d[2 * D] = s4.z;
      if (o0 + 3 < H) d[3 * D] = s4.w;
    }
  } else for (int e = threadIdx.x - 256; e < 9 * 32; e += HB_THREADS - 256) {
    const int k = e >> 5, ii = e & 31;
    const float* v0 = stage + HB_WAVES * 1024;
    float s0 = 0.f;
#pragma unroll
    for (int w = 0; w < HB_WAVES; ++w) s0 += v0[(w * 9 + k) * 64 + ii] + v0[(w * 9 + k) * 64 + 32 + ii];
    if (k == 0) { if (ii < H) dstp[b_off[0] + ii] = s0; }
    else if (k < 5) { if (ii < H) dstp[w_off[1] + (int64_t)(k - 1) * H + ii] = s0; }
    else if (ii == 0) dstp[b_off[1] + (k - 5)] = 0.25f * s0;
  }
}

bool ngm_hash_mlp_bwd_takes(const ngm_field_cfg& fc, const BwdProblem& q) {
  if (fc.encoding != NGM_ENC_PERMUTO || q.stash_kind != 2 || q.points || fc.skip_mode != NGM_SKIP_NO ||
      fc.matmul_mode == NGM_MATMUL_F32 || fc.num_layers != 1 || fc.dim_enc > 32 || fc.dim_hidden > 32 || fc.dim_enc <= 16 ||
      fc.dim_out != 4)
    return false;
  if (q.fused_comp && q.per_block % (HB_WAVES * 32)) return false;
  return (q.P + 64) * 128 < ((int64_t)1 << 32);
}
int ngm_launch_hash_mlp_bwd(const FieldBwdArgs& a, int blocks, hipStream_t st) {
  if (!ngm_hash_mlp_bwd_takes(a.fc, bwd_problem(a)) || !a.raytab || !a.stashB || !a.hash_dE) return NGM_E_INVALID;
  if (a.fused_comp ? (!a.rayseed || !a.hash_xyz) : !a.hash_xyz_ready) return NGM_E_INVALID;
  NgmProfScope prof_(NGM_K_FIELD_BWD, st);
  const size_t lds = (size_t)LdsHB::TOTAL * sizeof(float);
  if (a.fused_comp) {
    (void)hipFuncSetAttribute((const void*)k_hash_mlp_bwd<true>, hipFuncAttributeMaxDynamicSharedMemorySize, (int)lds);
    hipLaunchKernelGGL(k_hash_mlp_bwd<true>, dim3(blocks), dim3(HB_THREADS), lds, st, a);
  } else {
    (void)hipFuncSetAttribute((const void*)k_hash_mlp_bwd<false>, hipFuncAttributeMaxDynamicSharedMemorySize, (int)lds);
    hipLaunchKernelGGL(k_hash_mlp_bwd<false>, dim3(blocks), dim3(HB_THREADS), lds, st, a);
  }
  return 0;
}
```

### neural_graph_mapping_amd/csrc/ngm_launch.h

```cpp
#pragma once
#include <hip/hip_runtime.h>

#include "../../include/ngm_hip.h"
#include "ngm_adam.h"

#ifndef NGM_BLOCK
#define NGM_WAVE 64
#define NGM_BLOCK 256
#define NGM_WAVES_PER_BLOCK 4
#endif

struct PointsFwdArgs {
  ngm_field_cfg fc;
  ngm_params pr;
  int F;
  int64_t P;
  int64_t per_block;
  const float* points;
  const float* pos;
  const float* quat;
  float* out;
  float* act;
  int64_t act_layer_stride;
};

struct RenderFwdArgs {
  ngm_field_cfg fc;
  ngm_params pr;
  ngm_render_cfg rc;
  ngm_rays rays;
  ngm_targets tg;
  ngm_prediction pred;
  int has_targets;
  int S;
  int rays_per_block;
  int waves_per_block;
  int maxs;
  float* raytab;
  float4* stashA;
  float2* stashB;
  float* loss_partials;
  float* rayseed;
  float* act;
  int64_t act_layer_stride;
  int act_layers;
  const float* neus_sd;
  int64_t neus_sd_stride;
  unsigned long long* debug_cycles;
  const int32_t* num_active;
};

struct GradAdam {
  const ngm_adam_tensor* tensors;
  int num;
  AdamHyper hyper;
};
struct FieldBwdArgs {
  ngm_field_cfg fc;
  ngm_params pr;
  int F;
  int64_t P;
  int64_t per_block;
  int blocks_per_field;
  const float* points;
  const float* pos;
  const float* quat;
  const float* raytab;
  const float2* stashB;
  int S;
  const float4* d_out;
  float* partials;
  int64_t p_pad;
  float* lattice_grad;
  int64_t lattice_grad_stride;
  float2* hash_dE;
  float4* hash_xyz;
  float* hash_part;
  int hash_xyz_ready;
  long long* tri_acc;
  int64_t tri_numel;
  float* planes_grad;
  int64_t planes_grad_stride;
  const float* act;
  int64_t act_layer_stride;
  int act_half;
  unsigned long long* debug_cycles;
  GradAdam lattice_adam;
  int fused_comp;
  ngm_render_cfg rc;
  const float* rayseed;
  const float* loss_sums;
  const float* loss_partials; int n_partials;
  float* sums_out; float* loss_out; unsigned long long* counter;
  const int32_t* num_active;
};
struct BwdProblem {
  bool points;
  int64_t P, per_block;
  int stash_kind;
  bool half, fused_comp;
};
static inline BwdProblem bwd_problem(const FieldBwdArgs& a) {
  return {a.points != nullptr, a.P, a.per_block, a.act ? (a.fc.encoding == NGM_ENC_PERMUTO ? 2 : 1) : 0, a.act_half != 0, a.fused_comp != 0};
}
bool ngm_field_bwd_b3_takes(const ngm_field_cfg& fc, const BwdProblem& q);
bool ngm_hash_mlp_bwd_takes(const ngm_field_cfg& fc, const BwdProblem& q);
bool ngm_field_bwd16s_takes(const ngm_field_cfg& fc, const BwdProblem& q);
bool ngm_field_bwd16_takes(const ngm_field_cfg& fc, const BwdProblem& q);
bool ngm_field_bwd_takes(const ngm_field_cfg& fc, const BwdProblem& q);
struct GradReduceArgs;
bool ngm_hash_grad_takes(const ngm_field_cfg& fc);
int ngm_launch_hash_grad(const FieldBwdArgs& a, hipStream_t st, bool* adam_applied = nullptr, const GradReduceArgs* mlp_reduce = nullptr,
                         bool* mlp_reduced = nullptr);

struct GradReduceArgs {
  ngm_field_cfg fc;
  ngm_grads gr;
  int F;
  int blocks_per_field;
  const float* partials;
  int64_t p_pad;
  GradAdam adam;
  const int32_t* num_active = nullptr;
};

struct CompositeArgs {
  ngm_render_cfg rc;
  int64_t N;
  int S;
  const float* colors; const float* geoms; const float* dists; const float* depths; const float* isds;
  const float4* out4; const float* pcam; float* rgbd;
  const int* pair_field; const float* pair_w; const float4* pair_out; int pair_K; float outside_value; const float* ray_dir;
  float* C; float* D; float* Cv; float* Dv; float* term; float* weights;
  const float* dC; const float* dD; const float* dterm;
  float* d_colors; float* d_geoms; float* d_isds;
};

struct StashBwdArgs {
  ngm_render_cfg rc;
  int F, R, S;
  float4* stashA;
  const float2* stashB;
  const float* raytab;
  int seed_mode;
  ngm_targets tg;
  ngm_prediction pred;
  const float* loss_sums;
  const float* d_rgbds;
  const float* d_term;
  const float* d_geom_samples;
  const float* d_cvars;
  const float* d_dvars;
  float* loss_out;
  const float* neus_sd; int64_t neus_sd_stride; const int64_t* field_index;
  float4* d_out;
  float* d_isd_rays;
  const float* loss_partials;
  int n_partials;
  float* sums_out;
  unsigned long long* counter;
  float4* xyz_out;
  const int32_t* num_active;
};

#ifdef NGM_FAST_BUILD
#define NGM_FWD_SHAPES(X) X(2, 2, 2)
#else
#define NGM_FWD_SHAPES(X) X(2, 2, 2) X(2, 2, 1) X(1, 1, 1) X(1, 1, 2) X(2, 2, 3)
#endif
#define NGM_LDS_MAX (160 * 1024)
constexpr bool ngm_fwd_split_shape(int MI, int MH, int L) { return MI == 2 && MH == 2 && L <= 2; }
static inline bool ngm_fwd_split_takes(const ngm_field_cfg& fc) {
  return ngm_fwd_split_shape((fc.dim_enc + 31) / 32, (fc.dim_hidden + 31) / 32, fc.num_layers) && fc.skip_mode == NGM_SKIP_NO &&
         (fc.encoding == NGM_ENC_FOURIER || fc.encoding == NGM_ENC_NONE);
}
enum { NGM_FWD_RENDER = 0, NGM_FWD_POINTS = 1, NGM_FWD_KNN = 2 };
struct FwdPlan {
  int status = NGM_OK; const char* why = nullptr;
  int surface = NGM_FWD_RENDER;
  int MI = 0, MH = 0, L = 0;
  int matmul = -1;
  bool need_cos = false;
  int hash = 0, skip = 0;
  bool neus = false, one_tile = false, counted = false;
  int waves = 0, threads = 0;
  int rays_per_block = 0, maxs = 0;
  int64_t per_block = 0;
  int blocks = 0;
  int64_t lds_bytes = 0;
};
bool ngm_render_fwd_takes(const ngm_field_cfg& fc, bool neus, bool b3);
bool ngm_points_fwd_takes(const ngm_field_cfg& fc, bool b3);
bool ngm_knn_eval_takes(const ngm_field_cfg& fc, bool b3);
int64_t ngm_fwd_lds_bytes(const ngm_field_cfg& fc, bool b3, int waves, int maxs);
int ngm_launch_points_fwd(const PointsFwdArgs& a, const FwdPlan& p, hipStream_t st);
int64_t ngm_encode_bwd_fourier_scratch(int F, int64_t P);
int ngm_launch_encode_bwd_fourier(const ngm_field_cfg& fc, const ngm_params& pr, int F, int64_t P, const float* points,
                                  const float* pos, const float* quat, const float* d_enc, float* grad, int64_t grad_stride,
                                  float* scratch, hipStream_t st);
int ngm_launch_encode_bwd_prep_hash(const ngm_field_cfg& fc, const ngm_params& pr, int F, int64_t P, const float* points,
                                    const float* pos, const float* quat, const float* d_enc, float2* dE, float4* xyz,
                                    hipStream_t st);
int ngm_launch_encode_points(const ngm_field_cfg& fc, const ngm_params& pr, int F, int64_t P, const float* points, const float* pos,
                             const float* quat, float* out, hipStream_t st);
int ngm_launch_render_fwd(const RenderFwdArgs& a, const FwdPlan& p, hipStream_t st);
int ngm_launch_field_bwd(const FieldBwdArgs& a, int blocks, hipStream_t st);
int ngm_launch_tri_finish(const FieldBwdArgs& a, hipStream_t st);
int ngm_launch_field_bwd_b3(const FieldBwdArgs& a, int blocks, hipStream_t st);
int ngm_launch_hash_mlp_bwd(const FieldBwdArgs& a, int blocks, hipStream_t st);
int ngm_launch_field_bwd16s(const FieldBwdArgs& a, int blocks, hipStream_t st);
int ngm_launch_field_bwd16(const FieldBwdArgs& a, int blocks, hipStream_t st);
int ngm_launch_grad_reduce(const GradReduceArgs& a, hipStream_t st);
int ngm_launch_composite_fwd(const CompositeArgs& a, hipStream_t st);
int ngm_launch_composite_bwd(const CompositeArgs& a, hipStream_t st);
int ngm_launch_stash_bwd(const StashBwdArgs& a, hipStream_t st);
int ngm_launch_loss_exchange(const ngm_peer_exchange& px, float* sums, hipStream_t st);
double ngm_peer_set_timeout_impl(double seconds);
int ngm_peer_alloc_impl(int64_t bytes, void** out);

int ngm_launch_target_visibility(const ngm_keyframes& kf, int F, const float* field_pos, int num_offsets, const float* offsets,
                                 float radius, uint8_t* kf_mask, float* bbox, hipStream_t st);
int ngm_launch_target_sv_intersect(int F, int64_t N, const float* pos_c, const float* points, float radius, uint8_t* hit, hipStream_t st);
int ngm_launch_target_sv_rays(int F, int R, const float* pos_c, float radius, const int64_t* pts_ijs, const int64_t* segments,
                              const float* image, int height, int width, float fx, float fy, float cx, float cy, const ngm_target_out& o,
                              hipStream_t st);
int ngm_launch_target_rays(const ngm_keyframes& kf, int F, int R, const float* field_pos, float radius, const float* bbox,
                           const int64_t* frame_cids, const float* u_xy, const ngm_target_out& o, hipStream_t st);
int64_t ngm_target_sample_mv_bytes(int num_frames, int num_current, int num_fields, int capacity);
int ngm_launch_target_sample_mv(const ngm_keyframes& kf, const ngm_target_sample& s, const ngm_target_live* live ,
                                const ngm_target_out& o, void* workspace, int64_t workspace_bytes, hipStream_t st,
                                const int32_t* num_fields_dev = nullptr );
int64_t ngm_target_observed_fields_bytes(int height, int width);
int ngm_launch_target_observed_fields(const ngm_observed_fields& a, void* workspace, int64_t workspace_bytes, hipStream_t st,
                                      const int32_t* num_fields_dev = nullptr);
int ngm_launch_fields_append(const ngm_fields_append_args& a, hipStream_t st);
int ngm_launch_fields_repose(const ngm_fields_repose_args& a, hipStream_t st);
int ngm_launch_field_counts_add(const int64_t* field_ids, const int32_t* count, int rows, int num_fields, int64_t* training_iterations,
                                hipStream_t st);

__host__ __device__ static inline int64_t ngm_param_offsets(const ngm_field_cfg* fc, int64_t* enc_off, int64_t* w_off, int64_t* b_off) {
  int64_t o = 0;
  *enc_off = 0;
  if (fc->encoding == NGM_ENC_FOURIER) o += (int64_t)(fc->raw_coords ? fc->dim_enc - 3 : fc->dim_enc) * 3;
  for (int l = 0; l <= fc->num_layers; ++l) {
    const int din = (l == 0) ? fc->dim_enc : fc->dim_hidden + (fc->skip_mode == NGM_SKIP_CONCAT ? fc->dim_enc : 0);
    const int dout = (l == fc->num_layers) ? fc->dim_out : fc->dim_hidden;
    w_off[l] = o; o += (int64_t)din * dout;
    b_off[l] = o; o += dout;
  }
  return o;
}

struct NgmProfScope {
  int id; hipStream_t st; bool on;
  NgmProfScope(int kernel_id, hipStream_t stream);
  ~NgmProfScope();
};
```

Baseline: 2.411 billion ray-samples/s.

## Align gradient partial rows and vectorize grad-reduce and partial stores with float4

Adds a partial-buffer layout with a leading pad so each weight/bias segment starts 16-byte aligned, and records which segments can be accessed as float4. The grad-reduce kernel now sums four parameters per thread with float4 loads across block partials, and the bwd epilogue writes partials as float4 rows where the mask allows. The goal is fewer, wider memory transactions in the partial write and reduction. The cost is more complex segment lookup logic and a small padding overhead per row. Debug entry points for the layout and reduction are also added.

```diff
diff --git a/include/ngm_hip.h b/include/ngm_hip.h
--- a/include/ngm_hip.h
+++ b/include/ngm_hip.h
@@ -535,6 +535,12 @@
 int ngm_debug_plan_fwd(const ngm_field_cfg* fcfg, const ngm_render_cfg* rcfg, int32_t surface, int32_t F, int64_t n, int32_t guided,
                        int32_t* out12);
 
+int ngm_debug_partial_layout(const ngm_field_cfg* fcfg, int64_t* out, int32_t capacity);
+int ngm_debug_grad_reduce(const ngm_field_cfg* fcfg, const ngm_grads* grads, int32_t F, int32_t blocks_per_field, const float* partials,
+                          const ngm_adam_tensor* tensors, int32_t num_tensors, const int64_t* field_index, int64_t step, float lr,
+                          float beta1, float beta2, float eps, float weight_decay, const int32_t* num_active, int32_t* vec_mask_out,
+                          void* stream);
+
 #define NGM_MAX_PEERS 8
 typedef struct ngm_peer_exchange {
   int32_t world, rank;
diff --git a/neural_graph_mapping_amd/_capi.py b/neural_graph_mapping_amd/_capi.py
--- a/neural_graph_mapping_amd/_capi.py
+++ b/neural_graph_mapping_amd/_capi.py
@@ -371,6 +371,10 @@
     L.ngm_debug_plan_bwd.restype = C.c_int
     L.ngm_debug_plan_fwd.argtypes = [P(FieldCfg), P(RenderCfg), i32, i32, i64, i32, P(i32)]
     L.ngm_debug_plan_fwd.restype = C.c_int
+    L.ngm_debug_partial_layout.argtypes = [P(FieldCfg), P(i64), i32]
+    L.ngm_debug_partial_layout.restype = C.c_int
+    L.ngm_debug_grad_reduce.argtypes = [P(FieldCfg), P(Grads), i32, i32, vp, vp, i32, vp, i64, f32, f32, f32, f32, f32, vp, P(i32), vp]
+    L.ngm_debug_grad_reduce.restype = C.c_int
     L.ngm_profile_enable.argtypes = [i32]
     L.ngm_profile_read.argtypes = [i32, P(C.c_double), P(i64)]
     for name in ("ngm_profile_enable", "ngm_profile_reset", "ngm_profile_read"):
@@ -390,7 +394,7 @@
             "ngm_composite_fwd", "ngm_composite_bwd", "ngm_render_workspace", "ngm_render_fwd",
             "ngm_render_bwd", "ngm_render_bwd_adam", "ngm_render_bwd_seeded", "ngm_render_bwd_seeded_vars", "ngm_render_read_samples", "ngm_adam_sparse",
             "ngm_field_eval_knn", "ngm_field_eval_knn_workspace", "ngm_grid_eval_knn", "ngm_grid_eval_knn_workspace", "ngm_render_eval_knn", "ngm_render_eval_knn_workspace", "ngm_adam_sparse_multi", "ngm_step_advance", "ngm_profile_enable", "ngm_profile_reset", "ngm_profile_read",
-            "ngm_debug_phase_cycles", "ngm_debug_fwd_phase_cycles", "ngm_debug_last_bwd_variant", "ngm_debug_last_matmul", "ngm_debug_last_fwd_one_tile", "ngm_debug_last_comp_fused", "ngm_debug_disable_fused_comp", "ngm_debug_stash_mode", "ngm_debug_last_stash_mode", "ngm_debug_plan_bwd", "ngm_debug_plan_fwd", "ngm_target_visibility", "ngm_target_rays", "ngm_target_sv_intersect", "ngm_target_sv_rays",
+            "ngm_debug_phase_cycles", "ngm_debug_fwd_phase_cycles", "ngm_debug_last_bwd_variant", "ngm_debug_last_matmul", "ngm_debug_last_fwd_one_tile", "ngm_debug_last_comp_fused", "ngm_debug_disable_fused_comp", "ngm_debug_stash_mode", "ngm_debug_last_stash_mode", "ngm_debug_plan_bwd", "ngm_debug_plan_fwd", "ngm_debug_partial_layout", "ngm_debug_grad_reduce", "ngm_target_visibility", "ngm_target_rays", "ngm_target_sv_intersect", "ngm_target_sv_rays",
             "ngm_target_sample_mv_workspace", "ngm_target_sample_mv",
             "ngm_target_sample_mv_live_workspace", "ngm_target_sample_mv_live", "ngm_target_observed_fields_workspace",
             "ngm_target_observed_fields", "ngm_field_counts_add",
diff --git a/neural_graph_mapping_amd/csrc/ngm_api.hip b/neural_graph_mapping_amd/csrc/ngm_api.hip
--- a/neural_graph_mapping_amd/csrc/ngm_api.hip
+++ b/neural_graph_mapping_amd/csrc/ngm_api.hip
@@ -764,10 +764,7 @@
   return check_launch("ngm_encode_bwd");
 }
 
-static int64_t param_pad(const ngm_field_cfg* fc) {
-  int64_t e, w[NGM_MAX_LAYERS + 1], b[NGM_MAX_LAYERS + 1];
-  return align_up(ngm_param_offsets(fc, &e, w, b), 64);
-}
+static int64_t param_pad(const ngm_field_cfg* fc) { return ngm_partial_layout(fc).p_pad; }
 
 static void field_eval_bwd_layout(const ngm_field_cfg* fc, int64_t P, FieldBwdArgs& a, WsArena& ws) {
   a.partials = ws.take<float>((int64_t)a.F * a.blocks_per_field * a.p_pad + 64);
@@ -777,7 +774,7 @@
   if (check_field_cfg(fcfg)) return NGM_E_INVALID;
   FieldBwdArgs a = FieldBwdArgs();
   int64_t per;
-  a.F = F; a.p_pad = param_pad(fcfg);
+  a.F = F; ngm_set_partial_layout(fcfg, a);
   plan_bwd(F, P, &per, &a.blocks_per_field);
   return ws_bytes(field_eval_bwd_layout, fcfg, P, a);
 }
@@ -852,7 +849,7 @@
     a.act = field_eval_stash_layout(fcfg, F, P, &a.act_layer_stride, ss);
     if (!stash || !ss.covers(stash_bytes)) return fail(NGM_E_WORKSPACE, "ngm_field_eval_bwd_stash: stash too small");
   }
-  a.F = F; a.blocks_per_field = plan.blocks_per_field; a.p_pad = param_pad(fcfg);
+  a.F = F; a.blocks_per_field = plan.blocks_per_field; ngm_set_partial_layout(fcfg, a);
   WsArena ws(workspace);
   field_eval_bwd_layout(fcfg, P, a, ws);
   if (!ws.covers(workspace_bytes) || !workspace) return fail(NGM_E_WORKSPACE, "workspace too small");
@@ -1140,7 +1137,7 @@
   }
   a.per_block = p.bwd.per_block; a.blocks_per_field = p.bwd.blocks_per_field;
   a.raytab = sb.raytab; a.stashB = sb.stashB; a.d_out = neus ? sb.d_out : sb.stashA;
-  a.partials = reinterpret_cast<float*>(ws + p.off_gradpart); a.p_pad = p.p_pad;
+  a.partials = reinterpret_cast<float*>(ws + p.off_gradpart); ngm_set_partial_layout(fcfg, a);
   if (p.bwd.stash_kind) { a.act = reinterpret_cast<const float*>(ws + p.off_act); a.act_layer_stride = p.act_layer_stride; a.act_half = p.bwd.half; }
   if (p.bwd.fused_comp) {
     a.fused_comp = 1; a.rc = sb.rc;
@@ -1741,6 +1738,38 @@
   return p.status ? fail(p.status, p.why) : NGM_OK;
 }
 
+int ngm_debug_partial_layout(const ngm_field_cfg* fcfg, int64_t* out, int32_t capacity) {
+  const int e = check_field_cfg(fcfg);
+  if (e) return e;
+  const NgmPartialLayout y = ngm_partial_layout(fcfg);
+  if (!out || capacity < 5 + 2 * y.nseg) return fail(NGM_E_INVALID, "ngm_debug_partial_layout: out holds 5 + 2 x segments values");
+  out[0] = y.lead; out[1] = y.p_pad; out[2] = y.ptot; out[3] = y.nseg; out[4] = y.vec;
+  for (int k = 0; k < y.nseg; ++k) { out[5 + 2 * k] = y.off[k]; out[6 + 2 * k] = y.size[k]; }
+  return NGM_OK;
+}
+
+int ngm_debug_grad_reduce(const ngm_field_cfg* fcfg, const ngm_grads* grads, int32_t F, int32_t blocks_per_field, const float* partials,
+                          const ngm_adam_tensor* tensors, int32_t num_tensors, const int64_t* field_index, int64_t step, float lr,
+                          float beta1, float beta2, float eps, float weight_decay, const int32_t* num_active, int32_t* vec_mask_out,
+                          void* stream) {
+  const int e = check_field_cfg(fcfg);
+  if (e) return e;
+  if (!grads || !partials || F < 1 || blocks_per_field < 1 || (tensors && step < 1)) return fail(NGM_E_INVALID, "ngm_debug_grad_reduce: bad argument");
+  GradReduceArgs g;
+  memset(&g.adam, 0, sizeof(g.adam));
+  if (tensors) {
+    g.adam.tensors = tensors; g.adam.num = num_tensors;
+    g.adam.hyper = AdamHyper{field_index, nullptr, step, lr, beta1, beta2, eps, weight_decay};
+  }
+  g.num_active = num_active;
+  g.fc = *fcfg; g.gr = *grads; g.F = F; g.blocks_per_field = blocks_per_field; g.partials = partials; g.p_pad = param_pad(fcfg);
+  uint32_t vec = 0;
+  if (ngm_grad_reduce_vec_mask(g, &vec) || ngm_launch_grad_reduce(g, (hipStream_t)stream))
+    return fail(NGM_E_INVALID, "ngm_debug_grad_reduce: partials not 16-byte aligned, or adam tensors do not match the parameter segments");
+  if (vec_mask_out) *vec_mask_out = (int32_t)vec;
+  return check_launch("ngm_grad_reduce");
+}
+
 double ngm_peer_set_timeout(double seconds) { return ngm_peer_set_timeout_impl(seconds); }
 
 int ngm_loss_exchange(const ngm_peer_exchange* px, float* loss_sums, void* stream) {
diff --git a/neural_graph_mapping_amd/csrc/ngm_bwd16.h b/neural_graph_mapping_amd/csrc/ngm_bwd16.h
--- a/neural_graph_mapping_amd/csrc/ngm_bwd16.h
+++ b/neural_graph_mapping_amd/csrc/ngm_bwd16.h
@@ -511,7 +511,7 @@
   int64_t enc_off, w_off[NGM_MAX_LAYERS + 1], b_off[NGM_MAX_LAYERS + 1];
   const int64_t ptot = ngm_param_offsets(&a.fc, &enc_off, w_off, b_off);
   (void)ptot;
-  float* dst = a.partials + (int64_t)blockIdx.x * a.p_pad;
+  float* dst = ngm_partial_row(a, blockIdx.x);
   const int D = a.fc.dim_enc, H = a.fc.dim_hidden;
   constexpr int NT0 = TH * TI, NTH = TH * TH, NT = NT0 + (L - 1) * NTH;
   constexpr int EPI_W = EPI_CH * 4 * 64;
diff --git a/neural_graph_mapping_amd/csrc/ngm_field_bwd.hip b/neural_graph_mapping_amd/csrc/ngm_field_bwd.hip
--- a/neural_graph_mapping_amd/csrc/ngm_field_bwd.hip
+++ b/neural_graph_mapping_amd/csrc/ngm_field_bwd.hip
@@ -489,85 +489,168 @@
     }
     __syncthreads();
   }
-  float* dst = a.partials + (int64_t)blockIdx.x * a.p_pad;
+  float* dst = ngm_partial_row(a, blockIdx.x);
   for (int64_t p = threadIdx.x; p < ptot; p += NGM_BLOCK) dst[p] = red[p];
 }
 
-struct GradSeg { int64_t off, size; float* dst; int64_t stride; float* param; float* m; float* v; int64_t pstride; void* lp; int lp_dt; };
+struct GradSeg { int64_t off, size; float* dst; int64_t stride; float* param; float* m; float* v; int64_t pstride; void* lp; int lp_dt; int vec; };
 struct GradReduceK {
-  int F, blocks_per_field, nseg;
+  int F, blocks_per_field, nseg, any_lp;
   const float* partials;
-  int64_t p_pad, ptot;
-  GradSeg seg[2 * (NGM_MAX_LAYERS + 1) + 1];
+  int64_t p_pad, pend;
+  GradSeg seg[NGM_MAX_PARAM_SEGS];
   AdamHyper hyper;
   const int32_t* num_active;
 };
 
+struct GradQuad {
+  int seg[4];
+  bool vec;
+  float *D[4], *P[4], *M[4], *V[4];
+  float pv[4], m0[4], v0[4];
+};
+__device__ __forceinline__ int grad_seg_of(const GradReduceK& a, int64_t pp) {
+  for (int k = 0; k < a.nseg; ++k)
+    if (pp >= a.seg[k].off && pp < a.seg[k].off + a.seg[k].size) return k;
+  return -1;
+}
+__device__ __forceinline__ bool grad_quad_open(const GradReduceK& a, int f, int64_t pp, GradQuad& g) {
+  int k = -1;
+  int64_t end = 0;
+  float *d = nullptr, *p = nullptr, *m = nullptr, *v = nullptr;
+#pragma unroll
+  for (int e = 0; e < 4; ++e) {
+    const int64_t x = pp + e;
+    if (k >= 0 && x < end) {
+      if (d) ++d;
+      if (p) { ++p; ++m; ++v; }
+    } else {
+      k = grad_seg_of(a, x);
+      d = p = m = v = nullptr;
+      if (k >= 0) {
+        end = a.seg[k].off + a.seg[k].size;
+        const int64_t i = x - a.seg[k].off;
+        if (a.seg[k].dst) d = a.seg[k].dst + (int64_t)f * a.seg[k].stride + i;
+        if (a.seg[k].param) {
+          const int64_t row = a.hyper.field_index ? a.hyper.field_index[f] : f;
+          const int64_t so = row * a.seg[k].pstride + i;
+          p = a.seg[k].param + so; m = a.seg[k].m + so; v = a.seg[k].v + so;
+        }
+      }
+    }
+    g.seg[e] = k; g.D[e] = d; g.P[e] = p; g.M[e] = m; g.V[e] = v;
+    g.pv[e] = g.m0[e] = g.v0[e] = 0.f;
+  }
+  g.vec = g.seg[0] >= 0 && a.seg[g.seg[0]].vec;
+  if (g.vec) {
+    if (g.P[0]) {
+      const float4 p4 = *reinterpret_cast<const float4*>(g.P[0]), m4 = *reinterpret_cast<const float4*>(g.M[0]),
+                   v4 = *reinterpret_cast<const float4*>(g.V[0]);
+      g.pv[0] = p4.x; g.pv[1] = p4.y; g.pv[2] = p4.z; g.pv[3] = p4.w;
+      g.m0[0] = m4.x; g.m0[1] = m4.y; g.m0[2] = m4.z; g.m0[3] = m4.w;
+      g.v0[0] = v4.x; g.v0[1] = v4.y; g.v0[2] = v4.z; g.v0[3] = v4.w;
+    }
+  } else {
+#pragma unroll
+    for (int e = 0; e < 4; ++e)
+      if (g.P[e]) { g.pv[e] = *g.P[e]; g.m0[e] = *g.M[e]; g.v0[e] = *g.V[e]; }
+  }
+  return g.P[0] || g.P[1] || g.P[2] || g.P[3];
+}
+__device__ __forceinline__ void grad_quad_close(const GradReduceK& a, GradQuad& g, const float (&s)[4], const AdamCoef& co) {
+  float pn[4] = {0.f, 0.f, 0.f, 0.f};
+#pragma unroll
+  for (int e = 0; e < 4; ++e)
+    if (g.P[e]) pn[e] = adam_update(g.pv[e], g.m0[e], g.v0[e], s[e], co, a.hyper.beta1, a.hyper.beta2, a.hyper.eps, a.hyper.wd);
+  if (g.vec) {
+    if (g.D[0]) *reinterpret_cast<float4*>(g.D[0]) = make_float4(s[0], s[1], s[2], s[3]);
+    if (g.P[0]) {
+      *reinterpret_cast<float4*>(g.M[0]) = make_float4(g.m0[0], g.m0[1], g.m0[2], g.m0[3]);
+      *reinterpret_cast<float4*>(g.V[0]) = make_float4(g.v0[0], g.v0[1], g.v0[2], g.v0[3]);
+      *reinterpret_cast<float4*>(g.P[0]) = make_float4(pn[0], pn[1], pn[2], pn[3]);
+    }
+  } else {
+#pragma unroll
+    for (int e = 0; e < 4; ++e) {
+      if (g.D[e]) *g.D[e] = s[e];
+      if (g.P[e]) { *g.M[e] = g.m0[e]; *g.V[e] = g.v0[e]; *g.P[e] = pn[e]; }
+    }
+  }
+  if (a.any_lp) {
+#pragma unroll
+    for (int e = 0; e < 4; ++e)
+      if (g.P[e] && a.seg[g.seg[e]].lp) ngm_stp(a.seg[g.seg[e]].lp, g.P[e] - a.seg[g.seg[e]].param, pn[e], a.seg[g.seg[e]].lp_dt);
+  }
+}
+#define NGM_ADD4(S, V) do { S.x += V.x; S.y += V.y; S.z += V.z; S.w += V.w; } while (0)
+
 template <bool COUNTED>
 __global__ void __launch_bounds__(256) k_grad_reduce(GradReduceK a) {
-  __shared__ float part[4][64];
+  __shared__ float4 part[4][64];
   const int f = blockIdx.y, q = threadIdx.x >> 6, l = threadIdx.x & 63;
   if constexpr (COUNTED) {
     if (f >= *a.num_active) return;
   }
-  const int64_t p = (int64_t)blockIdx.x * 64 + l;
+  const int64_t pp = ((int64_t)blockIdx.x * 64 + l) * 4, px = (int64_t)blockIdx.x * 256 + threadIdx.x;
+  const bool live = pp < a.pend;
   int seg = -1;
   int64_t so = 0;
   float pv = 0.f, m0 = 0.f, v0 = 0.f;
   AdamCoef co = {0.f, 1.f};
-  const bool adam = q == 0 && p < a.ptot;
-  if (adam) {
-    for (int k = 0; k < a.nseg; ++k)
-      if (p >= a.seg[k].off && p < a.seg[k].off + a.seg[k].size) { seg = k; break; }
+  if (px < a.pend) {
+    seg = grad_seg_of(a, px);
     if (seg >= 0 && a.seg[seg].param) {
       const int64_t row = a.hyper.field_index ? a.hyper.field_index[f] : f;
-      so = row * a.seg[seg].pstride + (p - a.seg[seg].off);
+      so = row * a.seg[seg].pstride + (px - a.seg[seg].off);
       pv = a.seg[seg].param[so]; m0 = a.seg[seg].m[so]; v0 = a.seg[seg].v[so];
     }
   }
-  const float* src = a.partials + (int64_t)f * a.p_pad + p;
-  const int64_t cs = (int64_t)a.F * a.p_pad;
+  const bool adam = seg >= 0 && a.seg[seg].param;
+  const float4* src = reinterpret_cast<const float4*>(a.partials + (int64_t)f * a.p_pad + pp);
+  const int64_t cs = (int64_t)a.F * (a.p_pad >> 2);
   int c = q;
-  float v8[8] = {0.f, 0.f, 0.f, 0.f, 0.f, 0.f, 0.f, 0.f};
-  const bool pre = p < a.ptot && c + 28 < a.blocks_per_field;
+  const float4 z4 = make_float4(0.f, 0.f, 0.f, 0.f);
+  float4 v8[8] = {z4, z4, z4, z4, z4, z4, z4, z4};
+  const bool pre = live && c + 28 < a.blocks_per_field;
   if (pre) {
 #pragma unroll
     for (int j = 0; j < 8; ++j) v8[j] = src[(c + 4 * j) * cs];
   }
-  if (adam && seg >= 0 && a.seg[seg].param) {
+  if (adam) {
     const double step = (double)(a.hyper.step_dev ? *a.hyper.step_dev : a.hyper.step);
     co = adam_coef(a.hyper.lr, a.hyper.beta1, a.hyper.beta2, step);
   }
-  float s = 0.f;
+  float4 s = z4;
   if (pre) {
 #pragma unroll
-    for (int j = 0; j < 8; ++j) s += v8[j];
+    for (int j = 0; j < 8; ++j) NGM_ADD4(s, v8[j]);
     c += 32;
   }
-  if (p < a.ptot) {
+  if (live) {
 #pragma unroll 1
     for (; c + 28 < a.blocks_per_field; c += 32) {
-      float v[8];
+      float4 v[8];
 #pragma unroll
       for (int j = 0; j < 8; ++j) v[j] = src[(c + 4 * j) * cs];
 #pragma unroll
-      for (int j = 0; j < 8; ++j) s += v[j];
+      for (int j = 0; j < 8; ++j) NGM_ADD4(s, v[j]);
     }
 #pragma unroll 1
     for (; c + 12 < a.blocks_per_field; c += 16) {
-      const float v0_ = src[c * cs], v1 = src[(c + 4) * cs], v2 = src[(c + 8) * cs], v3 = src[(c + 12) * cs];
-      s += v0_; s += v1; s += v2; s += v3;
-    }
-    for (; c < a.blocks_per_field; c += 4) s += src[c * cs];
+      const float4 v0_ = src[c * cs], v1 = src[(c + 4) * cs], v2 = src[(c + 8) * cs], v3 = src[(c + 12) * cs];
+      NGM_ADD4(s, v0_); NGM_ADD4(s, v1); NGM_ADD4(s, v2); NGM_ADD4(s, v3);
+    }
+    for (; c < a.blocks_per_field; c += 4) { const float4 v = src[c * cs]; NGM_ADD4(s, v); }
   }
   part[q][l] = s;
   __syncthreads();
-  if (q != 0 || p >= a.ptot || seg < 0) return;
-  s = ((part[0][l] + part[1][l]) + part[2][l]) + part[3][l];
-  const int64_t i = p - a.seg[seg].off;
-  if (a.seg[seg].dst) a.seg[seg].dst[(int64_t)f * a.seg[seg].stride + i] = s;
-  if (a.seg[seg].param) {
-    const float pn = adam_update(pv, m0, v0, s, co, a.hyper.beta1, a.hyper.beta2, a.hyper.eps, a.hyper.wd);
+  if (seg < 0) return;
+  const float* pf = reinterpret_cast<const float*>(part);
+  const float r = ((pf[threadIdx.x] + pf[256 + threadIdx.x]) + pf[512 + threadIdx.x]) + pf[768 + threadIdx.x];
+  const int64_t i = px - a.seg[seg].off;
+  if (a.seg[seg].dst) a.seg[seg].dst[(int64_t)f * a.seg[seg].stride + i] = r;
+  if (adam) {
+    const float pn = adam_update(pv, m0, v0, r, co, a.hyper.beta1, a.hyper.beta2, a.hyper.eps, a.hyper.wd);
     a.seg[seg].m[so] = m0; a.seg[seg].v[so] = v0;
     a.seg[seg].param[so] = pn;
     if (a.seg[seg].lp) ngm_stp(a.seg[seg].lp, so, pn, a.seg[seg].lp_dt);
@@ -575,44 +658,37 @@
 }
 
 template <bool COUNTED>
-__device__ __forceinline__ void grad_reduce_one(const GradReduceK& a, int f, int64_t p) {
-  if (p >= a.ptot) return;
+__device__ __forceinline__ void grad_reduce_one(const GradReduceK& a, int f, int64_t quad) {
+  const int64_t pp = quad * 4;
+  if (pp >= a.pend) return;
   if constexpr (COUNTED) {
     if (f >= *a.num_active) return;
   }
-  int seg = -1;
-  for (int k = 0; k < a.nseg; ++k)
-    if (p >= a.seg[k].off && p < a.seg[k].off + a.seg[k].size) { seg = k; break; }
-  int64_t so = 0;
-  float pv = 0.f, m0 = 0.f, v0 = 0.f;
-  const bool adam = seg >= 0 && a.seg[seg].param;
-  if (adam) {
-    const int64_t row = a.hyper.field_index ? a.hyper.field_index[f] : f;
-    so = row * a.seg[seg].pstride + (p - a.seg[seg].off);
-    pv = a.seg[seg].param[so]; m0 = a.seg[seg].m[so]; v0 = a.seg[seg].v[so];
-  }
-  const float* src = a.partials + (int64_t)f * a.p_pad + p;
-  const int64_t cs = (int64_t)a.F * a.p_pad;
-  float q[4] = {0.f, 0.f, 0.f, 0.f};
+  GradQuad g;
+  const bool adam = grad_quad_open(a, f, pp, g);
+  const float4* src = reinterpret_cast<const float4*>(a.partials + (int64_t)f * a.p_pad + pp);
+  const int64_t cs = (int64_t)a.F * (a.p_pad >> 2);
+  const float4 z4 = make_float4(0.f, 0.f, 0.f, 0.f);
+  float4 q[4] = {z4, z4, z4, z4};
   if (a.blocks_per_field <= 8) {
-    float v[8];
-#pragma unroll
-    for (int c = 0; c < 8; ++c) v[c] = (c < a.blocks_per_field) ? src[c * cs] : 0.f;
+    float4 v[8];
+#pragma unroll
+    for (int c = 0; c < 8; ++c) v[c] = (c < a.blocks_per_field) ? src[c * cs] : z4;
 #pragma unroll
     for (int i = 0; i < 4; ++i) {
-      float s = 0.f;
-      if (i < a.blocks_per_field) s += v[i];
-      if (i + 4 < a.blocks_per_field) s += v[i + 4];
+      float4 s = z4;
+      if (i < a.blocks_per_field) NGM_ADD4(s, v[i]);
+      if (i + 4 < a.blocks_per_field) NGM_ADD4(s, v[i + 4]);
       q[i] = s;
     }
   } else {
     for (int c0 = 0; c0 < a.blocks_per_field; c0 += 16) {
-      float v[16];
-#pragma unroll
-      for (int u = 0; u < 16; ++u) v[u] = (c0 + u < a.blocks_per_field) ? src[(int64_t)(c0 + u) * cs] : 0.f;
+      float4 v[16];
+#pragma unroll
+      for (int u = 0; u < 16; ++u) v[u] = (c0 + u < a.blocks_per_field) ? src[(int64_t)(c0 + u) * cs] : z4;
 #pragma unroll
       for (int u = 0; u < 16; ++u)
-        if (c0 + u < a.blocks_per_field) q[u & 3] += v[u];
+        if (c0 + u < a.blocks_per_field) NGM_ADD4(q[u & 3], v[u]);
     }
   }
   AdamCoef co = {0.f, 1.f};
@@ -620,64 +696,72 @@
     const double step = (double)(a.hyper.step_dev ? *a.hyper.step_dev : a.hyper.step);
     co = adam_coef(a.hyper.lr, a.hyper.beta1, a.hyper.beta2, step);
   }
-  const float s = ((q[0] + q[1]) + q[2]) + q[3];
-  if (seg < 0) return;
-  const int64_t i = p - a.seg[seg].off;
-  if (a.seg[seg].dst) a.seg[seg].dst[(int64_t)f * a.seg[seg].stride + i] = s;
-  if (adam) {
-    const float pn = adam_update(pv, m0, v0, s, co, a.hyper.beta1, a.hyper.beta2, a.hyper.eps, a.hyper.wd);
-    a.seg[seg].m[so] = m0; a.seg[seg].v[so] = v0;
-    a.seg[seg].param[so] = pn;
-    if (a.seg[seg].lp) ngm_stp(a.seg[seg].lp, so, pn, a.seg[seg].lp_dt);
-  }
+  const float r[4] = {((q[0].x + q[1].x) + q[2].x) + q[3].x, ((q[0].y + q[1].y) + q[2].y) + q[3].y, ((q[0].z + q[1].z) + q[2].z) + q[3].z,
+                      ((q[0].w + q[1].w) + q[2].w) + q[3].w};
+  grad_quad_close(a, g, r, co);
 }
 template <bool COUNTED>
 __global__ void __launch_bounds__(256) k_grad_reduce_flat(GradReduceK a) {
   grad_reduce_one<COUNTED>(a, blockIdx.y, (int64_t)blockIdx.x * 256 + threadIdx.x);
 }
-
+#undef NGM_ADD4
+
+static bool aligned16(const void* p) { return (reinterpret_cast<uintptr_t>(p) & 15) == 0; }
 static int build_grad_reduce(const GradReduceArgs& g, GradReduceK& k) {
+  const NgmPartialLayout y = ngm_partial_layout(&g.fc);
+  if (g.p_pad != y.p_pad || !aligned16(g.partials)) return NGM_E_INVALID;
   k.F = g.F; k.blocks_per_field = g.blocks_per_field; k.partials = g.partials; k.p_pad = g.p_pad;
   k.num_active = g.num_active;
-  int64_t enc_off, w_off[NGM_MAX_LAYERS + 1], b_off[NGM_MAX_LAYERS + 1];
-  k.ptot = ngm_param_offsets(&g.fc, &enc_off, w_off, b_off);
-  int n = 0;
-  if (g.fc.encoding == NGM_ENC_FOURIER) {
-    const int64_t sz = (int64_t)(g.fc.raw_coords ? g.fc.dim_enc - 3 : g.fc.dim_enc) * 3;
-    k.seg[n++] = GradSeg{enc_off, sz, g.gr.enc_w, g.gr.enc_w_stride, nullptr, nullptr, nullptr, 0, nullptr, 0};
-  }
+  k.pend = y.lead + y.ptot;
+  const int n = y.nseg;
+  int i = 0;
+  if (y.has_enc) { k.seg[i] = GradSeg{y.off[i], y.size[i], g.gr.enc_w, g.gr.enc_w_stride, nullptr, nullptr, nullptr, 0, nullptr, 0, 0}; ++i; }
   for (int l = 0; l <= g.fc.num_layers; ++l) {
-    const int din = (l == 0) ? g.fc.dim_enc : g.fc.dim_hidden + (g.fc.skip_mode == NGM_SKIP_CONCAT ? g.fc.dim_enc : 0);
-    const int dout = (l == g.fc.num_layers) ? g.fc.dim_out : g.fc.dim_hidden;
-    k.seg[n++] = GradSeg{w_off[l], (int64_t)din * dout, g.gr.w[l], g.gr.w_stride[l], nullptr, nullptr, nullptr, 0, nullptr, 0};
-    k.seg[n++] = GradSeg{b_off[l], (int64_t)dout, g.gr.b[l], g.gr.b_stride[l], nullptr, nullptr, nullptr, 0, nullptr, 0};
+    k.seg[i] = GradSeg{y.off[i], y.size[i], g.gr.w[l], g.gr.w_stride[l], nullptr, nullptr, nullptr, 0, nullptr, 0, 0}; ++i;
+    k.seg[i] = GradSeg{y.off[i], y.size[i], g.gr.b[l], g.gr.b_stride[l], nullptr, nullptr, nullptr, 0, nullptr, 0, 0}; ++i;
   }
   k.nseg = n;
   k.hyper = AdamHyper{nullptr, nullptr, 1, 0.f, 0.f, 0.f, 0.f, 0.f};
   if (g.adam.tensors) {
     if (g.adam.num != n) return NGM_E_INVALID;
-    for (int i = 0; i < n; ++i) {
-      const ngm_adam_tensor& t = g.adam.tensors[i];
-      if (t.numel != k.seg[i].size || !t.param || !t.exp_avg || !t.exp_avg_sq) return NGM_E_INVALID;
-      k.seg[i].param = t.param; k.seg[i].m = t.exp_avg; k.seg[i].v = t.exp_avg_sq; k.seg[i].pstride = t.stride;
-      k.seg[i].lp = t.param_lp; k.seg[i].lp_dt = t.lp_dtype;
+    for (int j = 0; j < n; ++j) {
+      const ngm_adam_tensor& t = g.adam.tensors[j];
+      if (t.numel != k.seg[j].size || !t.param || !t.exp_avg || !t.exp_avg_sq) return NGM_E_INVALID;
+      k.seg[j].param = t.param; k.seg[j].m = t.exp_avg; k.seg[j].v = t.exp_avg_sq; k.seg[j].pstride = t.stride;
+      k.seg[j].lp = t.param_lp; k.seg[j].lp_dt = t.lp_dtype;
     }
     k.hyper = g.adam.hyper;
   }
+  k.any_lp = 0;
+  for (int j = 0; j < n; ++j) {
+    const GradSeg& s = k.seg[j];
+    if (s.lp) k.any_lp = 1;
+    k.seg[j].vec = ((y.vec >> j) & 1u) && (!s.dst || (aligned16(s.dst) && s.stride % 4 == 0)) &&
+                   (!s.param || (aligned16(s.param) && aligned16(s.m) && aligned16(s.v) && s.pstride % 4 == 0));
+  }
   return 0;
+}
+static int ngm_grad_reduce_quads(const GradReduceK& k) { return (int)((k.pend + 3) / 4); }
+int ngm_grad_reduce_vec_mask(const GradReduceArgs& g, uint32_t* mask) {
+  GradReduceK k;
+  const int rc = build_grad_reduce(g, k);
+  *mask = 0;
+  for (int j = 0; !rc && j < k.nseg; ++j) *mask |= (uint32_t)k.seg[j].vec << j;
+  return rc;
 }
 int ngm_launch_grad_reduce(const GradReduceArgs& g, hipStream_t st) {
   NgmProfScope prof_(NGM_K_GRAD_REDUCE, st);
   GradReduceK k;
   const int rc = build_grad_reduce(g, k);
   if (rc) return rc;
+  const int quads = ngm_grad_reduce_quads(k);
   if (k.blocks_per_field <= 8) {
-    dim3 grid((unsigned)((k.ptot + 255) / 256), (unsigned)g.F);
+    dim3 grid((unsigned)((quads + 255) / 256), (unsigned)g.F);
     if (k.num_active) hipLaunchKernelGGL(k_grad_reduce_flat<true>, grid, dim3(256), 0, st, k);
     else hipLaunchKernelGGL(k_grad_reduce_flat<false>, grid, dim3(256), 0, st, k);
     return 0;
   }
-  dim3 grid((unsigned)((k.ptot + 63) / 64), (unsigned)g.F);
+  dim3 grid((unsigned)((quads + 63) / 64), (unsigned)g.F);
   if (k.num_active) hipLaunchKernelGGL(k_grad_reduce<true>, grid, dim3(256), 0, st, k);
   else hipLaunchKernelGGL(k_grad_reduce<false>, grid, dim3(256), 0, st, k);
   return 0;
@@ -1027,7 +1111,7 @@
   a.hash_blocks = chunks * units;
   if (mlp_reduce) {
     if (build_grad_reduce(*mlp_reduce, a.mlp)) return NGM_E_INVALID;
-    a.mlp_bx = (int)((a.mlp.ptot + NT - 1) / NT);
+    a.mlp_bx = (ngm_grad_reduce_quads(a.mlp) + NT - 1) / NT;
     if (mlp_reduced) *mlp_reduced = true;
   }
   const int grid_x = a.hash_blocks + a.mlp_bx * (int)fb.F;
diff --git a/neural_graph_mapping_amd/csrc/ngm_field_bwd_b3.hip b/neural_graph_mapping_amd/csrc/ngm_field_bwd_b3.hip
--- a/neural_graph_mapping_amd/csrc/ngm_field_bwd_b3.hip
+++ b/neural_graph_mapping_amd/csrc/ngm_field_bwd_b3.hip
@@ -667,18 +667,20 @@
   constexpr int NV = 2 * L + 8 + 6 + 4;
   static_assert(LY::EPI_ACC + B3B_WAVES * NV * 64 <= LY::TOTAL, "the per-feature vectors are staged behind the accumulator tiles");
   float* stagev = sm + LY::EPI_ACC;
-#pragma unroll
-  for (int l = 0; l < L; ++l)
-#pragma unroll
-    for (int mo = 0; mo < 2; ++mo)
-#pragma unroll
-      for (int mi = 0; mi < 2; ++mi)
-#pragma unroll
-        for (int q = 0; q < 4; ++q) {
+  {
+    const int ec = lane & 31, ehi = lane >> 5;
+#pragma unroll
+    for (int l = 0; l < L; ++l)
+#pragma unroll
+      for (int mo = 0; mo < 2; ++mo)
+#pragma unroll
+        for (int mi = 0; mi < 2; ++mi) {
           const f32x16& c = acc[l][mo][mi];
-          *reinterpret_cast<float4*>(stage + (((wave * NT + (l * 4 + mo * 2 + mi)) * 4 + q) * 64 + lane) * 4) =
-              make_float4(c[4 * q], c[4 * q + 1], c[4 * q + 2], c[4 * q + 3]);
-        }
+          float* st = stage + (wave * NT + (l * 4 + mo * 2 + mi)) * 1024 + 128 * ehi + ec;
+#pragma unroll
+          for (int r = 0; r < 16; ++r) st[(8 * (r >> 2) + (r & 3)) * 32] = c[r];
+        }
+  }
   {
     float* sw = stagev + wave * NV * 64;
     int k = 0;
@@ -700,11 +702,12 @@
   __syncthreads();
   int64_t enc_off, w_off[NGM_MAX_LAYERS + 1], b_off[NGM_MAX_LAYERS + 1];
   (void)ngm_param_offsets(&a.fc, &enc_off, w_off, b_off);
-  float* dst = a.partials + (int64_t)blockIdx.x * a.p_pad;
+  float* dst = ngm_partial_row(a, blockIdx.x);
   const int D = a.fc.dim_enc, H = a.fc.dim_hidden;
+  const uint32_t vmask = a.partial_vec >> a.partial_seg0;
   {
-    static_assert(NT * 256 % B3B_THREADS == 0, "whole passes");
-    constexpr int NIT = NT * 256 / B3B_THREADS;
+    static_assert(NT * 256 == NT * B3B_THREADS, "one accumulator tile per pass");
+    constexpr int NIT = NT;
     float4 v4[NIT][B3B_WAVES];
 #pragma unroll
     for (int it = 0; it < NIT; ++it)
@@ -713,55 +716,65 @@
         v4[it][w] = *reinterpret_cast<const float4*>(stage + (w * NT * 256 + it * B3B_THREADS + threadIdx.x) * 4);
 #pragma unroll
     for (int it = 0; it < NIT; ++it) {
-      const int e4 = it * B3B_THREADS + threadIdx.x;
       float4 s4 = make_float4(0.f, 0.f, 0.f, 0.f);
 #pragma unroll
       for (int w = 0; w < B3B_WAVES; ++w) {
         s4.x += v4[it][w].x; s4.y += v4[it][w].y; s4.z += v4[it][w].z; s4.w += v4[it][w].w;
       }
-      const int t = e4 >> 8, q = (e4 >> 6) & 3, ln = e4 & 63;
-      const int l = t >> 2, mo = (t >> 1) & 1, mi = t & 1;
-      const int o0 = 32 * mo + 8 * q + 4 * (ln >> 5), c = 32 * mi + (ln & 31), din = (l == 0) ? D : H;
-      if (c < din) {
-        float* d = dst + w_off[l] + (int64_t)o0 * din + c;
-        if (o0 < H) d[0] = s4.x;
-        if (o0 + 1 < H) d[din] = s4.y;
-        if (o0 + 2 < H) d[2 * din] = s4.z;
-        if (o0 + 3 < H) d[3 * din] = s4.w;
+      const int l = it >> 2, mo = (it >> 1) & 1, mi = it & 1;
+      const int o = 32 * mo + (threadIdx.x >> 3), c0 = 32 * mi + 4 * (threadIdx.x & 7), din = (l == 0) ? D : H;
+      if (o < H && c0 < din) {
+        float* d = dst + w_off[l] + (int64_t)o * din + c0;
+        if ((vmask >> (2 * l)) & 1u) ngm_store_wt(reinterpret_cast<float4*>(d), s4);
+        else {
+          d[0] = s4.x;
+          if (c0 + 1 < din) d[1] = s4.y;
+          if (c0 + 2 < din) d[2] = s4.z;
+          if (c0 + 3 < din) d[3] = s4.w;
+        }
       }
     }
   }
   const bool fourier = ENC_GRAD && a.fc.encoding == NGM_ENC_FOURIER;
   const int n_raw = a.fc.raw_coords ? 3 : 0;
   {
-    constexpr int NIV = (NV * 32 + B3B_THREADS - 1) / B3B_THREADS;
-    float sv[NIV];
-#pragma unroll
-    for (int it = 0; it < NIV; ++it) {
-      const int e = it * B3B_THREADS + threadIdx.x;
-      const int k = min(e >> 5, NV - 1), ii = e & 31;
-      float s0 = 0.f;
-#pragma unroll
-      for (int w = 0; w < B3B_WAVES; ++w) s0 += stagev[(w * NV + k) * 64 + ii] + stagev[(w * NV + k) * 64 + 32 + ii];
-      sv[it] = s0;
-    }
-#pragma unroll
-    for (int it = 0; it < NIV; ++it) {
-      const int e = it * B3B_THREADS + threadIdx.x;
-      if (e >= NV * 32) break;
-      const int k = e >> 5, ii = e & 31;
-      const float s0 = sv[it];
-      if (k < 2 * L) {
-        const int l = k >> 1, ft = 32 * (k & 1) + ii;
-        if (ft < H) dst[b_off[l] + ft] = s0;
-      } else if (k < 2 * L + 8) {
-        const int u = k - 2 * L, ft = 32 * (u >> 2) + ii, c = u & 3;
-        if (ft < H) dst[w_off[L] + (int64_t)c * H + ft] = s0;
+    constexpr int NQ = NV * 8;
+    static_assert(NQ <= B3B_THREADS && (2 * L + 14) * 8 % 64 + 32 <= 64, "one pass; the four output-bias sums sit in one wave");
+    if (threadIdx.x < NQ) {
+      const int k = threadIdx.x >> 3, i4 = 4 * (threadIdx.x & 7);
+      float4 lo[B3B_WAVES], hi[B3B_WAVES];
+#pragma unroll
+      for (int w = 0; w < B3B_WAVES; ++w) {
+        lo[w] = *reinterpret_cast<const float4*>(stagev + (w * NV + k) * 64 + i4);
+        hi[w] = *reinterpret_cast<const float4*>(stagev + (w * NV + k) * 64 + 32 + i4);
+      }
+      float4 s = make_float4(0.f, 0.f, 0.f, 0.f);
+#pragma unroll
+      for (int w = 0; w < B3B_WAVES; ++w) {
+        s.x += lo[w].x + hi[w].x; s.y += lo[w].y + hi[w].y; s.z += lo[w].z + hi[w].z; s.w += lo[w].w + hi[w].w;
+      }
+      const float ob1 = __shfl_down(s.x, 8, 64), ob2 = __shfl_down(s.x, 16, 64), ob3 = __shfl_down(s.x, 24, 64);
+      const float sv[4] = {s.x, s.y, s.z, s.w};
+      if (k < 2 * L + 8) {
+        const int u = k - 2 * L;
+        const int l = (k < 2 * L) ? (k >> 1) : L, ft = (k < 2 * L) ? 32 * (k & 1) + i4 : 32 * (u >> 2) + i4;
+        float* d = dst + ((k < 2 * L) ? b_off[l] : w_off[L] + (int64_t)(u & 3) * H) + ft;
+        const bool vec = (k < 2 * L) ? ((vmask >> (2 * l + 1)) & 1u) : ((vmask >> (2 * L)) & 1u);
+        if (vec) { if (ft < H) ngm_store_wt(reinterpret_cast<float4*>(d), s); }
+        else {
+#pragma unroll
+          for (int e = 0; e < 4; ++e) if (ft + e < H) d[e] = sv[e];
+        }
       } else if (k < 2 * L + 14) {
-        const int u = k - 2 * L - 8, ft = 32 * (u / 3) + ii, c = u % 3;
-        if (fourier && ft < D && ft >= n_raw) dst[enc_off + (int64_t)(ft - n_raw) * 3 + c] = s0;
-      } else if (ii == 0) {
-        dst[b_off[L] + (k - 2 * L - 14)] = 0.5f * s0;
+        const int u = k - 2 * L - 8, ft = 32 * (u / 3) + i4, c = u % 3;
+#pragma unroll
+        for (int e = 0; e < 4; ++e)
+          if (fourier && ft + e < D && ft + e >= n_raw) dst[enc_off + (int64_t)(ft + e - n_raw) * 3 + c] = sv[e];
+      } else if (k == 2 * L + 14 && i4 == 0) {
+        const float4 ob = make_float4(0.5f * s.x, 0.5f * ob1, 0.5f * ob2, 0.5f * ob3);
+        float* d = dst + b_off[L];
+        if ((vmask >> (2 * L + 1)) & 1u) ngm_store_wt(reinterpret_cast<float4*>(d), ob);
+        else { d[0] = ob.x; d[1] = ob.y; d[2] = ob.z; d[3] = ob.w; }
       }
     }
   }
diff --git a/neural_graph_mapping_amd/csrc/ngm_hash_bwd.hip b/neural_graph_mapping_amd/csrc/ngm_hash_bwd.hip
--- a/neural_graph_mapping_amd/csrc/ngm_hash_bwd.hip
+++ b/neural_graph_mapping_amd/csrc/ngm_hash_bwd.hip
@@ -393,7 +393,7 @@
   __syncthreads();
   int64_t enc_off, w_off[NGM_MAX_LAYERS + 1], b_off[NGM_MAX_LAYERS + 1];
   (void)ngm_param_offsets(&a.fc, &enc_off, w_off, b_off);
-  float* dstp = a.partials + (int64_t)blockIdx.x * a.p_pad;
+  float* dstp = ngm_partial_row(a, blockIdx.x);
   if (threadIdx.x < 256) {
     const int e4 = threadIdx.x;
     float4 s4 = make_float4(0.f, 0.f, 0.f, 0.f);
diff --git a/neural_graph_mapping_amd/csrc/ngm_launch.h b/neural_graph_mapping_amd/csrc/ngm_launch.h
--- a/neural_graph_mapping_amd/csrc/ngm_launch.h
+++ b/neural_graph_mapping_amd/csrc/ngm_launch.h
@@ -93,6 +93,8 @@
   const float* loss_partials; int n_partials;
   float* sums_out; float* loss_out; unsigned long long* counter;
   const int32_t* num_active;
+  int p_lead, partial_seg0;
+  uint32_t partial_vec;
 };
 struct BwdProblem {
   bool points;
@@ -211,6 +213,7 @@
 int ngm_launch_field_bwd16s(const FieldBwdArgs& a, int blocks, hipStream_t st);
 int ngm_launch_field_bwd16(const FieldBwdArgs& a, int blocks, hipStream_t st);
 int ngm_launch_grad_reduce(const GradReduceArgs& a, hipStream_t st);
+int ngm_grad_reduce_vec_mask(const GradReduceArgs& a, uint32_t* mask);
 int ngm_launch_composite_fwd(const CompositeArgs& a, hipStream_t st);
 int ngm_launch_composite_bwd(const CompositeArgs& a, hipStream_t st);
 int ngm_launch_stash_bwd(const StashBwdArgs& a, hipStream_t st);
@@ -251,6 +254,41 @@
   return o;
 }
 
+#define NGM_MAX_PARAM_SEGS (2 * (NGM_MAX_LAYERS + 1) + 1)
+struct NgmPartialLayout {
+  int lead, nseg, has_enc;
+  int64_t ptot, p_pad;
+  int64_t off[NGM_MAX_PARAM_SEGS], size[NGM_MAX_PARAM_SEGS];
+  uint32_t vec;
+};
+static inline NgmPartialLayout ngm_partial_layout(const ngm_field_cfg* fc) {
+  NgmPartialLayout y = NgmPartialLayout();
+  int64_t enc_off, w_off[NGM_MAX_LAYERS + 1], b_off[NGM_MAX_LAYERS + 1];
+  y.ptot = ngm_param_offsets(fc, &enc_off, w_off, b_off);
+  y.lead = (int)((4 - w_off[0] % 4) % 4);
+  y.p_pad = (y.lead + y.ptot + 63) / 64 * 64;
+  y.has_enc = fc->encoding == NGM_ENC_FOURIER;
+  int n = 0;
+  if (y.has_enc) { y.off[n] = y.lead + enc_off; y.size[n] = w_off[0] - enc_off; if (y.off[n] % 4 == 0 && y.size[n] % 4 == 0) y.vec |= 1u << n; ++n; }
+  for (int l = 0; l <= fc->num_layers; ++l) {
+    const int64_t din = (b_off[l] - w_off[l]) / ((l == fc->num_layers) ? fc->dim_out : fc->dim_hidden);
+    const int64_t end = (l == fc->num_layers) ? y.ptot : w_off[l + 1];
+    y.off[n] = y.lead + w_off[l]; y.size[n] = b_off[l] - w_off[l];
+    if (y.off[n] % 4 == 0 && y.size[n] % 4 == 0 && din % 4 == 0) y.vec |= 1u << n;
+    ++n;
+    y.off[n] = y.lead + b_off[l]; y.size[n] = end - b_off[l];
+    if (y.off[n] % 4 == 0 && y.size[n] % 4 == 0) y.vec |= 1u << n;
+    ++n;
+  }
+  y.nseg = n;
+  return y;
+}
+static inline void ngm_set_partial_layout(const ngm_field_cfg* fc, FieldBwdArgs& a) {
+  const NgmPartialLayout y = ngm_partial_layout(fc);
+  a.p_pad = y.p_pad; a.p_lead = y.lead; a.partial_vec = y.vec; a.partial_seg0 = y.has_enc;
+}
+__device__ __forceinline__ float* ngm_partial_row(const FieldBwdArgs& a, int64_t b) { return a.partials + b * a.p_pad + a.p_lead; }
+
 struct NgmProfScope {
   int id; hipStream_t st; bool on;
   NgmProfScope(int kernel_id, hipStream_t stream);
```

Result: no change. 2.412 billion ray-samples/s (median of 5 runs) (+0.0%).
